# nikhilTkur/Multigrid_Nikhil_C-

Hardware: AMD Instinct MI355X
Metric: fine_grid_stencil_updates_per_sec (higher is better)
Workload: dtype f64

## Files before the change

### multigrid_nikhil_c-_amd/csrc/mgx.hip

```cpp

#include "../../include/mgx.h"
#include "mgx_bottom.hpp"
#include "mgx_kernels.hpp"
#include "mgx_launch.hpp"
#include "mgx_var.hpp"
#include "mgx_galerkin.hpp"
#include "mgx_opdep.hpp"
#include "mgx_cheby.hpp"
#include "mgx_line.hpp"
#include "mgx_small.hpp"
#include "mgx_krylov.hpp"
#include "mgx_dist_plan.hpp"

#include <chrono>
#include <unistd.h>
#include <cmath>
#include <cstdio>
#include <cstdlib>
#include <cstring>
#include <string>
#include <vector>

namespace {

using namespace mgx;

thread_local std::string g_create_error;

void log_runtime_libs(const char* where)
{
    if (env_int("MGX_LOG_RUNTIME_LIBS", 0) == 0) return;
    char buf[8192];
    if (mgx_runtime_libs(buf, sizeof buf) >= 0)
        std::fprintf(stderr, "[mgx] runtime libraries mapped at %s (pid %d):\n%s", where, (int)getpid(), buf);
}

struct Level {
    int L = 0, N = 0, rows = 0;
    long pitch = 0;
    size_t bytes = 0;
    bool f64 = true;
    void *u = nullptr, *b = nullptr, *tmp = nullptr, *r = nullptr;
    void* A[9] = {};
    void* J[9] = {};
    void* wt[8] = {nullptr, nullptr, nullptr, nullptr, nullptr, nullptr, nullptr, nullptr};
    bool nine = false;
    bool stencil_set = false;
    void* cheb = nullptr;
    double lambda_g = 0.0;
    void *line_m[2] = {nullptr, nullptr}, *line_g[2] = {nullptr, nullptr}, *line_hf = nullptr, *line_hb = nullptr;
    int line_R = 0;
    size_t esize() const { return f64 ? 8 : 4; }
};

struct EventPair { hipEvent_t a, b; int cls; long long launches; long long sweeps; hipEvent_t a_use; };

}

struct mgx_solver {
    mgx_config cfg{};
    hipStream_t stream = nullptr;
    std::vector<Level> lv;
    Level fine64;
    bool mixed = false;
    bool work_f64 = true;
    BottomDST bottom;
    double* partial = nullptr;
    long partial_cap = 0;
    double* sum_dev = nullptr;
    double* sum_host = nullptr;
    std::string err;
    int rows_per_chunk = 0;
    FuseCfg fuse{10, 0, 256, 10, 10, 1024, 10, 10};
    std::vector<EventPair> ev_used, ev_free;
    double prof_ms[MGX_PROF_COUNT] = {0};
    long long prof_launches[MGX_PROF_COUNT] = {0};
    long long prof_sweeps[MGX_PROF_COUNT] = {0};
    int last_smooth_launches = 0;
    int fold = 1;
    int use_zero_in = 1;
    int norm_blocks_ready = 0;
    double fine_updates = 0.0;
    struct CycleGraph {
        std::vector<void*> before, after;
        hipGraphExec_t exec = nullptr;
        double fine_updates = 0.0;
    };
    std::vector<CycleGraph> graphs;
    int use_graph = 1;
    bool prof_mute = false;
    bool prof_chain = false;
    hipEvent_t chain_ev = nullptr;
    int mixed_fuse = 1;
    double *var_M = nullptr, *var_inv = nullptr, *var_pm = nullptr, *var_pi = nullptr;
    bool var = false;
    bool galerkin = false;
    bool gal_built = false;
    int cycle = MGX_CYCLE_V;
    int small_visit = 1;
    int small_max_n = kSmallMaxN;
    int line_dirs = 0;
    int* line_flag = nullptr;
    int transfer = MGX_TRANSFER_BILINEAR;
    struct KrylovWs {
        void *x = nullptr, *b = nullptr;
        void *p[2] = {nullptr, nullptr}, *q = nullptr;
        void *Z[kGcrMaxRestart] = {}, *Q[kGcrMaxRestart] = {};
        double* part = nullptr;
        long part_cap = 0;
        double *sc = nullptr, *sc_host = nullptr;
        int vecs(mgx_solver* s, std::initializer_list<void**> vs, size_t bytes);
        int shared(mgx_solver* s, size_t bytes, int blocks);
        void free();
    } kry;
    struct mgx_dist* dist = nullptr;

    int fail(int code, const std::string& m) { err = m; return code; }
};

namespace {

#define HIPCHK(h, expr)                                                                  \
    do {                                                                                 \
        hipError_t e__ = (expr);                                                         \
        if (e__ != hipSuccess)                                                           \
            return (h)->fail(MGX_ERR_HIP, std::string(#expr) + ": " + hipGetErrorString(e__)); \
    } while (0)

struct Prof {
    mgx_solver* s; int idx = -1;
    Prof(mgx_solver* s_, int cls, long long launches) : s(s_)
    {
        static const bool mute_all = env_int("MGX_PROF_MUTE", 0) != 0;
        if (!s->cfg.profile || s->prof_mute || mute_all) return;
        EventPair p;
        if (!s->ev_free.empty()) { p = s->ev_free.back(); s->ev_free.pop_back(); }
        else {
            static const unsigned flags = env_int("MGX_PROF_EVENT_FLAGS", 1) ? hipEventDisableSystemFence : hipEventDefault;
            if (hipEventCreateWithFlags(&p.a, flags) != hipSuccess || hipEventCreateWithFlags(&p.b, flags) != hipSuccess) return;
        }
        p.cls = cls; p.launches = launches; p.sweeps = 0;
        p.a_use = p.a;
        if (s->prof_chain && s->chain_ev) p.a_use = s->chain_ev;
        else (void)hipEventRecord(p.a, s->stream);
        s->ev_used.push_back(p);
        idx = (int)s->ev_used.size() - 1;
    }
    void set(long long launches, long long sweeps)
    {
        if (idx >= 0) { s->ev_used[idx].launches = launches; s->ev_used[idx].sweeps = sweeps; }
    }
    ~Prof()
    {
        if (idx < 0) return;
        (void)hipEventRecord(s->ev_used[idx].b, s->stream);
        if (s->prof_chain) s->chain_ev = s->ev_used[idx].b;
    }
};

int prof_collect(mgx_solver* s)
{
    if (s->ev_used.empty()) return MGX_OK;
    HIPCHK(s, hipStreamSynchronize(s->stream));
    for (auto& p : s->ev_used) {
// ... 300 lines not shown
    s->gal_built = true;
    s->transfer = transfer;
    drop_graphs(s);
    return MGX_OK;
}

void galerkin_invalidate(mgx_solver* s)
{
    for (int lv = s->cfg.coarsest_level; lv < s->cfg.finest_level; ++lv) s->lv[lv].stencil_set = false;
    s->lv[s->cfg.finest_level].stencil_set = true;
    s->gal_built = false;
    drop_graphs(s);
}

int var_ready(mgx_solver* s, int lo, int hi)
{
    if (!s->var) return MGX_OK;
    if (s->galerkin && !s->gal_built)
        return s->fail(MGX_ERR_STATE, s->lv[s->cfg.finest_level].stencil_set ? "Galerkin hierarchy not built (mgx_build_galerkin)"
                                                                             : "finest operator not set (mgx_set_stencil / mgx_set_coefficient)");
    for (int l = lo; l <= hi; ++l)
        if (!s->lv[l].stencil_set)
            return s->fail(MGX_ERR_STATE, "operator of level " + std::to_string(l) + " not set (mgx_set_stencil / mgx_set_coefficient)");
    return MGX_OK;
}

template <typename T>
void smooth_var_t(mgx_solver* s, Level& l, int mu)
{
    const T om = (T)s->cfg.omega;
    const T rc = (T)(1.0 - (double)om);
    const Launch g = make_launch(l.N, VecOf<T>::W, l.N - 1, 1);
    const VarLevel<T> v = var_level<T>(l);
    for (int i = 0; i < mu; ++i) {
        with_point_count(v.nine, [&](auto nq) {
            hipLaunchKernelGGL((k_jacobi_var<T, decltype(nq)::value>), dim3(g.blocks), dim3(kBlock), 0, s->stream, (const T*)l.u, (const T*)l.b,
                               (T*)l.tmp, v.dinv, v.r, v.N, v.pitch, 1, v.N, g.strips, rc, om, v.rows);
        });
        std::swap(l.u, l.tmp);
    }
    s->last_smooth_launches = mu;
}

template <typename T>
void smooth_cheby_t(mgx_solver* s, Level& l, int mu)
{
    const T om = (T)s->cfg.omega;
    const T rc = (T)(1.0 - (double)om);
    const std::vector<ChebyStep> st = cheby_scalars(s->cfg.omega, l.lambda_g, mu);
    const VarLevel<T> cl = var_level<T>(l);
    for (int i = 0; i < mu; ++i) {
        launch_cheby<T>(cl, (const T*)l.u, (const T*)l.b, (T*)l.tmp, (T*)l.cheb, i == 0, rc, om, (T)st[i].a, (T)st[i].c, s->stream);
        std::swap(l.u, l.tmp);
    }
    s->last_smooth_launches = mu;
}

template <typename T>
void smooth_line_t(mgx_solver* s, Level& l, int mu)
{
    const LineLevel<T> ll = line_level<T>(l);
    int launches = 0;
    for (int i = 0; i < mu; ++i) launches += launch_line_sweep<T>(ll, (T*)l.u, (const T*)l.b, s->line_dirs, s->stream);
    s->last_smooth_launches = launches;
}

void smooth_var(mgx_solver* s, Level& l, int mu)
{
    if (s->line_dirs) { if (l.f64) smooth_line_t<double>(s, l, mu); else smooth_line_t<float>(s, l, mu); }
    else if (s->cfg.smoother == MGX_SMOOTHER_CHEBYSHEV) { if (l.f64) smooth_cheby_t<double>(s, l, mu); else smooth_cheby_t<float>(s, l, mu); }
    else if (l.f64) smooth_var_t<double>(s, l, mu);
    else smooth_var_t<float>(s, l, mu);
}

template <typename T, int MODE>
void residual_var_t(mgx_solver* s, const Level& l, const void* u, const void* b, void* out)
{
    const Launch g = make_launch(l.N, VecOf<T>::W, l.N - 1, 1);
    const VarLevel<T> v = var_level<T>(l);
    with_point_count(v.nine, [&](auto nq) {
        hipLaunchKernelGGL((k_residual_var<T, decltype(nq)::value, MODE>), dim3(g.blocks), dim3(kBlock), 0, s->stream, (const T*)u, (const T*)b,
                           (T*)out, s->partial, v.a, v.N, v.pitch, 1, v.N, g.strips, v.rows);
    });
    if (MODE == 1) hipLaunchKernelGGL(k_reduce_partials, dim3(1), dim3(kReduceThreads), 0, s->stream, s->partial, g.blocks, s->sum_dev);
}

template <int MODE>
void residual_level(mgx_solver* s, const Level& l, const void* u, const void* b, void* out)
{
    with_float_type(l.f64, [&](auto tag) {
        using T = decltype(tag);
        if (s->var) residual_var_t<T, MODE>(s, l, u, b, out);
        else launch_residual<T, MODE>((const T*)u, (const T*)b, out, MODE ? 0 : l.pitch, MODE ? s->partial : nullptr, MODE ? s->sum_dev : nullptr,
                                      1.0, l.N, l.pitch, 1, l.N, s->rows_per_chunk, s->stream, MODE ? s->partial_cap : -1, l.rows);
    });
}

template <typename T, int SM, int AR>
int fold_block(const FuseCfg& fc, const BlockReq& q, T* u, const T* b, T* tmp, long pitch, double omega, const mgx_slab* c,
               const T* coarse_e, T* coarse_b, T* coarse_zero, int crow_lo, int crow_hi, int restrict_mode, double* partial,
               hipStream_t st, int* flips)
{
    std::vector<Pass> plan;
    if (!fold_plan(fc, q, &plan)) return -1;
    const int N = q.N, row0 = q.row0;
    const JacobiCoef<T> jc = jacobi_coef<T>(omega);
    FoldArgs fa;
    fa.restrict_mode = restrict_mode;
    fa.partial = partial;
    fa.win.row_first = std::max(row0, 0);
    fa.win.row_last = std::min(row0 + q.rows - 1, N);
    fa.win.crow_first = 0; fa.win.crow_last = -1; fa.win.emit_lo = 0; fa.win.emit_hi = 0;
    if (c) {
        fa.cpitch = level_pitch(c->level, c->dtype);
        fa.win.crow_first = std::max(c->row0, 0);
        fa.win.crow_last = std::min(c->row0 + c->rows - 1, N / 2);
        fa.win.emit_lo = std::max(c->row0 + crow_lo, 1);
        fa.win.emit_hi = std::min(c->row0 + crow_hi, N / 2);
        const long cback = (long)c->row0 * fa.cpitch;
        if (coarse_e) fa.coarse_e = coarse_e - cback;
        if (coarse_b) fa.coarse_b = coarse_b - cback;
        if (coarse_zero) fa.coarse_zero = coarse_zero - cback;
    }
    const long back = (long)row0 * pitch;
    T* src = u; T* dst = tmp;
    int blocks = 0;
    for (const Pass& p : plan) {
        if (p.hi > p.lo) {
            const int lo = p.lo - row0, hi = p.hi - row0;
            fa.row_lo = p.lo; fa.row_hi = p.hi;
            fa.zero_in = p.zero_in ? 1 : 0;
            int rc = 0;
            if (p.kind == PASS_JACOBI)
                rc = launch_jacobi<T>(src, b, dst, N, pitch, lo, hi, omega, p.R, st, q.rows, AR) ? -1 : 0;
            else if (p.kind == PASS_RBGS)
                launch_rbgs<T>(src, b, dst, N, pitch, lo, hi, row0 & 1, -row0, N - row0, p.R, st);
            else if (p.kind == PASS_FUSED)
                rc = launch_fused<T, SM, AR>(p.K, src, b, dst, N, pitch, lo, hi, jc.c0, jc.c1, -row0, N - row0, row0 & 1, p.R, st,
                                             q.rows, fa.zero_in) ? 0 : -1;
            else if (p.kind == PASS_FOLDED)
                rc = with_stages(p.pre, p.post, [&](auto s) {
                    using S = decltype(s);
                    if constexpr (S::PRE || S::POST)
                        return launch_cycle<T, S::PRE, S::POST, SM, AR>(p.K, src - back, b - back, dst - back, fa, N, pitch, jc.c0, jc.c1, p.R, st);
                    else
                        return -1;
                });
            else
                rc = launch_tile_pass<T, SM, AR>(src - back, b - back, dst - back, fa, N, pitch, jc.c0, jc.c1, p.K, p.R, p.pre, p.post, st);
            if (rc < 0) return -1;
            if (p.post == 2) blocks = rc;
        }
        std::swap(src, dst);
    }
    *flips = (int)plan.size();
    return blocks;
}

bool fold_eligible(const mgx_solver* s, const Level& l, int mu, bool pre = false, int post = 1, bool zero_in = false)
{
    if (!s->fold || mu < 1 || mu > 64) return false;
    if (s->var || (post == 1 && s->cfg.restrict_mode >= MGX_RESTRICT_INJECT)) return false;
    const int per = (s->cfg.smoother == MGX_SMOOTHER_RBGS) ? 2 : 1;
    if (!tile_level(s, l) && (l.N < s->fuse.min_n || s->fuse.kmax < per)) return false;
    std::vector<Pass> plan;
    return fold_plan(s->fuse, level_req(s, l, mu, pre, post, zero_in, 0), &plan);
}

bool zero_in_ok(const mgx_solver* s, int level)
{
    if (!s->use_zero_in || level <= s->cfg.coarsest_level) return false;
    return fold_eligible(s, s->lv[level], s->cfg.mu1, false, 1, true);
}

bool smooth_folded(mgx_solver* s, int level, int mu, bool pre, int post, bool zero_in = false, bool coarse_zero_in = false)
{
    Level& l = s->lv[level];
    if (!fold_eligible(s, l, mu, pre, post)) return false;
    const bool fine = (level == s->cfg.finest_level);
    const bool rbgs = (s->cfg.smoother == MGX_SMOOTHER_RBGS);
    if (!l.f64 && !rbgs && mu == 10 && l.N > s->fuse.tile_max_n && post == 2 && pre &&
        cycle_k_supported(mu, false, false, 0, pre, s->fuse.arith) && !cycle_k_supported(mu, false, false, post, pre, s->fuse.arith))
        post = 0;
    {
        Prof p(s, fine ? MGX_PROF_SMOOTH_FINE : MGX_PROF_COARSE, mu);
        const Level& c = s->lv[level - 1];
        const int dt = l.f64 ? MGX_DTYPE_F64 : MGX_DTYPE_F32;
        const mgx_slab cs{level - 1, dt, c.rows, 0, s->cfg.arith};
        void* czero = (post == 1 && coarse_zero_in) ? nullptr : c.u;
        const BlockReq q = level_req(s, l, mu, pre, post, zero_in, env_int("MGX_ROWS", 0));
        int launches = 0;
        const int nb = with_kernel_set(l.f64, s->cfg.smoother, s->fuse.arith, [&](auto k) {
            using K = decltype(k);
            using T = typename K::T;
            return fold_block<T, K::SM, K::AR>(s->fuse, q, (T*)l.u, (const T*)l.b, (T*)l.tmp, l.pitch, s->cfg.omega, &cs,
                                               pre ? (const T*)c.u : nullptr, post == 1 ? (T*)c.b : nullptr, (T*)czero, 1, c.N,
                                               s->cfg.restrict_mode, s->partial, s->stream, &launches);
        });
        if (nb < 0) return false;
        if (launches & 1) std::swap(l.u, l.tmp);
        p.set(launches, mu);
        if (post == 2) s->norm_blocks_ready = nb;
    }
    if (fine) s->fine_updates += (double)mu * (double)(l.N - 1) * (double)(l.N - 1);
    return true;
}

void smooth_t(mgx_solver* s, Level& l, int mu)
{
    int launches = 0;
    with_kernel_set(l.f64, s->cfg.smoother, s->fuse.arith, [&](auto k) {
        using K = decltype(k);
        using T = typename K::T;
        (void)fold_block<T, K::SM, K::AR>(s->fuse, level_req(s, l, mu, false, 0, false, s->rows_per_chunk), (T*)l.u, (const T*)l.b,
                                          (T*)l.tmp, l.pitch, s->cfg.omega, nullptr, nullptr, nullptr, nullptr, 0, 0, 0, nullptr,
                                          s->stream, &launches);
    });
    s->last_smooth_launches = launches;
    if (launches & 1) std::swap(l.u, l.tmp);
}

void smooth(mgx_solver* s, int level, int mu)
{
    if (mu <= 0) return;
    Level& l = s->lv[level];
    const bool fine = (level == s->cfg.finest_level);
    Prof p(s, fine ? MGX_PROF_SMOOTH_FINE : MGX_PROF_COARSE, mu);
    if (s->var) smooth_var(s, l, mu);
    else smooth_t(s, l, mu);
    p.set(s->last_smooth_launches, mu);
    if (fine) s->fine_updates += (double)(s->line_dirs == 3 ? 2 * mu : mu) * (double)(l.N - 1) * (double)(l.N - 1);
}

void restrict_level(mgx_solver* s, int level, bool fused, bool zero_guess)
{
    Level& f = s->lv[level];
    Level& c = s->lv[level - 1];
    const bool fine = (level == s->cfg.finest_level);
    Prof p(s, fine ? MGX_PROF_RESTRICT_FINE : MGX_PROF_COARSE, 1);
    const int rpc = s->rows_per_chunk;
    const int mode = s->cfg.restrict_mode;
    with_float_type(f.f64, [&](auto tag) {
        using T = decltype(tag);
        T* cz = zero_guess ? (T*)c.u : nullptr;
        if (opdep(s)) {
            const Launch g = make_launch(c.N, VecOf<T>::W, c.N - 1, 1);
            const T rscale = (mode == MGX_RESTRICT_FW16) ? (T)0.25 : (T)1;
            const dim3 grd(g.blocks), blk(kBlock);
            if (!fused) hipLaunchKernelGGL((k_restrict_opdep<T, 0>), grd, blk, 0, s->stream, (const T*)f.u, (const T*)f.b, op9_of<T>(f), wt8_of<T>(c),
                                           (T*)c.b, cz, c.N, f.pitch, c.pitch, g.strips, rscale);
            else with_point_count(f.nine, [&](auto nq) {
                hipLaunchKernelGGL((k_restrict_opdep<T, decltype(nq)::value == 9 ? 2 : 1>), grd, blk, 0, s->stream, (const T*)f.u, (const T*)f.b,
                                   op9_of<T>(f), wt8_of<T>(c), (T*)c.b, cz, c.N, f.pitch, c.pitch, g.strips, rscale);
            });
            return;
        }
        const bool grid_residual = fused && (s->var || mode >= MGX_RESTRICT_INJECT);
        if (grid_residual) residual_level<0>(s, f, f.u, f.b, f.r);
        const T* src = (const T*)(grid_residual ? f.r : f.b);
        if (mode >= MGX_RESTRICT_INJECT) {
            const double w = (mode == MGX_RESTRICT_INJECT4) ? 4.0 : 1.0;
            const dim3 blk(256), grd((c.N + 255) / 256, c.N - 1);
            hipLaunchKernelGGL((k_restrict_inject<T>), grd, blk, 0, s->stream, src, (T*)c.b, cz, c.N, f.pitch, c.pitch, (T)w);
        } else {
            launch_restrict<T>((const T*)f.u, src, (T*)c.b, cz, f.N, f.pitch, c.pitch, 1, c.N, 0, mode, fused && !grid_residual, rpc, s->stream);
        }
    });
}

void prolong_level(mgx_solver* s, int level, bool add)
{
    Level& f = s->lv[level];
    Level& c = s->lv[level - 1];
    const bool fine = (level == s->cfg.finest_level);
    Prof p(s, fine ? MGX_PROF_PROLONG_FINE : MGX_PROF_COARSE, 1);
    with_float_type(f.f64, [&](auto tag) {
        using T = decltype(tag);
        if (!opdep(s)) {
            launch_prolong<T>((T*)f.u, (const T*)c.u, f.N, f.pitch, c.pitch, 1, f.N, 0, add, s->rows_per_chunk, s->stream);
            return;
        }
        const Launch g = make_launch(c.N, VecOf<T>::W, c.N, 1);
        if (add) hipLaunchKernelGGL((k_prolong_opdep<T, true>), dim3(g.blocks), dim3(kBlock), 0, s->stream, (T*)f.u, (const T*)c.u, wt8_of<T>(c),
                                    c.N, f.pitch, c.pitch, g.strips);
        else hipLaunchKernelGGL((k_prolong_opdep<T, false>), dim3(g.blocks), dim3(kBlock), 0, s->stream, (T*)f.u, (const T*)c.u, wt8_of<T>(c),
                                c.N, f.pitch, c.pitch, g.strips);
    });
}

void bottom_solve(mgx_solver* s)
{
    Level& l = s->lv[s->cfg.coarsest_level];
    Prof p(s, (l.L == s->cfg.finest_level) ? MGX_PROF_SMOOTH_FINE : MGX_PROF_COARSE, 4);
    const int n = l.N - 1;
    with_float_type(l.f64, [&](auto tag) {
        using T = decltype(tag);
        if (s->var)
            hipLaunchKernelGGL((k_var_dense_solve<T>), dim3((n * n + 63) / 64), dim3(64), 0, s->stream, s->var_inv, (const T*)l.b, (T*)l.u, n, l.pitch);
        else s->bottom.solve<T>((const T*)l.b, (T*)l.u, l.pitch, s->stream);
    });
}

int zero_u(mgx_solver* s, int level)
{
    Level& l = s->lv[level];
    HIPCHK(s, hipMemsetAsync(l.u, 0, l.bytes, s->stream));
    return MGX_OK;
}

bool descend(mgx_solver* s, int level, bool zero_in_here)
{
    const bool zin_next = zero_in_ok(s, level - 1);
    if (!smooth_folded(s, level, s->cfg.mu1, false, 1, zero_in_here, zin_next)) {
        if (zero_in_here) (void)zero_u(s, level);
        smooth(s, level, s->cfg.mu1);
        restrict_level(s, level, true, !zin_next);
    }
    return zin_next;
}

void ascend(mgx_solver* s, int level, int post)
{
    if (!smooth_folded(s, level, s->cfg.mu2, true, post)) {
        prolong_level(s, level, true);
        smooth(s, level, s->cfg.mu2);
    }
}

void vcycle(mgx_solver* s, int level, bool zero_in_here = false, int post_top = 0, int kind = -1);

bool small_level(const mgx_solver* s, int level)
{
    if (!s->small_visit || s->cycle == MGX_CYCLE_V || !s->galerkin || !s->gal_built) return false;
    if (s->cfg.smoother != MGX_SMOOTHER_JACOBI) return false;
    if (level <= s->cfg.coarsest_level || level > s->cfg.finest_level) return false;
    const Level& l = s->lv[level];
    return l.nine && l.N <= s->small_max_n;
}

void small_visit(mgx_solver* s, int level, bool ascend, bool descend)
{
    Level& f = s->lv[level];
    Level& c = s->lv[level - 1];
    Prof p(s, MGX_PROF_COARSE, 1);
    with_float_type(f.f64, [&](auto tag) {
        using T = decltype(tag);
        SmallVisit<T> a;
        a.u = (T*)f.u; a.b = (const T*)f.b;
        a.a = op9_of<T>(f); a.r = jac9_of<T>(f); a.dinv = (const T*)f.J[0];
        a.cu = (T*)c.u; a.cb = (T*)c.b;
        a.w = wt8_of<T>(c);
        a.N = f.N; a.pitch = f.pitch; a.cpitch = c.pitch;
        a.ascend = ascend; a.descend = descend; a.mu1 = s->cfg.mu1; a.mu2 = s->cfg.mu2;
        a.opdep = opdep(s);
        a.omega = (T)s->cfg.omega;
        a.rc = (T)(1.0 - (double)a.omega);
        const bool fw16 = s->cfg.restrict_mode == MGX_RESTRICT_FW16;
        a.rscale = fw16 ? (T)0.25 : (T)1;
        a.wgt = fw16 ? (T)0.0625 : (T)0.25;
        launch_small_visit<T>(a, s->stream);
    });
    p.set(1, (ascend ? s->cfg.mu2 : 0) + (descend ? s->cfg.mu1 : 0));
}

void coarse_visits(mgx_solver* s, int level, bool zero_in_here, int kind)
{
    const bool twice = kind != MGX_CYCLE_V && level > s->cfg.coarsest_level;
    const int second = kind == MGX_CYCLE_F ? MGX_CYCLE_V : kind;
    if (twice && small_level(s, level)) {
        small_visit(s, level, false, true);
        coarse_visits(s, level - 1, false, kind);
        small_visit(s, level, true, true);
        coarse_visits(s, level - 1, false, second);
        small_visit(s, level, true, false);
        return;
    }
    vcycle(s, level, zero_in_here, 0, kind);
    if (twice) vcycle(s, level, false, 0, second);
}

void vcycle(mgx_solver* s, int level, bool zero_in_here, int post_top, int kind)
{
    if (kind < 0) kind = s->cycle;
    if (level == s->cfg.coarsest_level) {
        if (s->cfg.bottom == MGX_BOTTOM_EXACT) {
            bottom_solve(s);
        } else {
            smooth(s, level, s->cfg.mu1);
            smooth(s, level, s->cfg.mu2);
        }
        return;
    }
    if (small_level(s, level)) {
        small_visit(s, level, false, true);
        coarse_visits(s, level - 1, false, kind);
        small_visit(s, level, true, false);
        return;
    }
    const bool zin_next = descend(s, level, zero_in_here);
    coarse_visits(s, level - 1, zin_next, kind);
    ascend(s, level, post_top);
}

int fmg(mgx_solver* s)
{
    const int lo = s->cfg.coarsest_level, hi = s->cfg.finest_level;
    for (int l = hi; l > lo; --l) restrict_level(s, l, false, false);
    if (s->cfg.bottom == MGX_BOTTOM_EXACT) {
        bottom_solve(s);
    } else {
        int rc = zero_u(s, lo);
        if (rc) return rc;
        for (int i = 0; i <= s->cfg.mu0; ++i) vcycle(s, lo);
    }
    for (int l = lo + 1; l <= hi; ++l) {
        prolong_level(s, l, false);
        for (int i = 0; i <= s->cfg.mu0; ++i) vcycle(s, l);
    }
    return MGX_OK;
}

int enqueue_norm(mgx_solver* s, const Level& l, const void* u, const void* b, int cls)
{
    if (s->norm_blocks_ready > 0 && u == s->lv[s->cfg.finest_level].u && !s->mixed) {
        Prof p(s, cls, 1);
        hipLaunchKernelGGL(k_reduce_partials, dim3(1), dim3(kReduceThreads), 0, s->stream, s->partial, s->norm_blocks_ready,
                           s->sum_dev);
    } else {
        Prof p(s, cls, 2);
        residual_level<1>(s, l, u, b, nullptr);
    }
    s->norm_blocks_ready = 0;
    HIPCHK(s, hipMemcpyAsync(s->sum_host, s->sum_dev, sizeof(double), hipMemcpyDeviceToHost, s->stream));
    return MGX_OK;
}

int residual_norm_grid(mgx_solver* s, const Level& l, const void* u, const void* b, double* out, int cls)
{
    int rc = enqueue_norm(s, l, u, b, cls);
    if (rc) return rc;
    HIPCHK(s, hipStreamSynchronize(s->stream));
    *out = std::sqrt(*s->sum_host);
    return MGX_OK;
}

constexpr size_t kMaxGraphs = 8;

std::vector<void*> buffer_state(const mgx_solver* s)
{
    std::vector<void*> v;
    for (int l = s->cfg.coarsest_level; l <= s->cfg.finest_level; ++l) { v.push_back(s->lv[l].u); v.push_back(s->lv[l].tmp); }
    return v;
}

void set_buffer_state(mgx_solver* s, const std::vector<void*>& v)
{
    size_t i = 0;
    for (int l = s->cfg.coarsest_level; l <= s->cfg.finest_level; ++l) { s->lv[l].u = v[i++]; s->lv[l].tmp = v[i++]; }
}

template <typename Body>
hipGraphExec_t cached_graph(mgx_solver* s, unsigned tag, Body&& enqueue)
{
    std::vector<void*> key = buffer_state(s);
    key.push_back(reinterpret_cast<void*>((uintptr_t)tag));
    for (auto& c : s->graphs)
        if (c.before == key) {
            set_buffer_state(s, c.after);
            s->fine_updates += c.fine_updates;
            return c.exec;
        }
    if (s->graphs.size() >= kMaxGraphs) return nullptr;
    const double fu0 = s->fine_updates;
    hipGraph_t graph = nullptr;
    hipGraphExec_t exec = nullptr;
    hipError_t e = hipStreamBeginCapture(s->stream, hipStreamCaptureModeThreadLocal);
    if (e == hipSuccess) {
        s->prof_mute = true;
        const int rc = enqueue();
        s->prof_mute = false;
        e = hipStreamEndCapture(s->stream, &graph);
        if (e == hipSuccess && rc != MGX_OK) e = hipErrorUnknown;
        if (e == hipSuccess) e = hipGraphInstantiate(&exec, graph, nullptr, nullptr, 0);
        if (graph) (void)hipGraphDestroy(graph);
    }
    if (e != hipSuccess) {
        (void)hipGetLastError();
        set_buffer_state(s, key);
        s->fine_updates = fu0;
        s->use_graph = 0;
        return nullptr;
    }
    s->graphs.push_back({key, buffer_state(s), exec, s->fine_updates - fu0});
    return exec;
}

int coarse_part_graph(mgx_solver* s, int level, bool zero_in_here)
{
    auto body = [&] { coarse_visits(s, level, zero_in_here, s->cycle); return MGX_OK; };
    const hipGraphExec_t exec = cached_graph(s, 4u | (zero_in_here ? 8u : 0u), body);
    if (!exec) return body();
    Prof p(s, MGX_PROF_COARSE, 1);
    HIPCHK(s, hipGraphLaunch(exec, s->stream));
    return MGX_OK;
}

int zero_start_u(mgx_solver* s, bool* implicit)
{
    const int L = s->cfg.finest_level;
    const bool one_level = L == s->cfg.coarsest_level;
    *implicit = zero_in_ok(s, L);
    if (*implicit) return MGX_OK;
    if (one_level && !s->mixed) return MGX_OK;
    return zero_u(s, L);
}

int enqueue_cycle(mgx_solver* s, bool want_norm, bool zero_start, bool split)
{
    struct Chain {
        mgx_solver* s;
        Chain(mgx_solver* s_, bool on) : s(s_) { s->prof_chain = on && env_int("MGX_PROF_CHAIN", 1) != 0; s->chain_ev = nullptr; }
        ~Chain() { s->prof_chain = false; s->chain_ev = nullptr; }
    } chain(s, split);
    const int L = s->cfg.finest_level;
    const int post = want_norm ? 2 : 0;
    s->norm_blocks_ready = 0;
    bool zin = false;
    if (zero_start)
        if (int rc = zero_start_u(s, &zin)) return rc;
    if (split) {
        const bool zin_next = descend(s, L, zin);
        if (int rc = coarse_part_graph(s, L - 1, zin_next)) return rc;
        ascend(s, L, post);
    } else {
        vcycle(s, L, zin, post);
    }
    return want_norm ? enqueue_norm(s, s->lv[L], s->lv[L].u, s->lv[L].b, MGX_PROF_NORM_FINE) : MGX_OK;
}

int cycle_body(mgx_solver* s, bool want_norm, bool zero_start, double* r)
{
    const bool split = s->cfg.profile == 2 && s->use_graph && !s->mixed && s->cfg.finest_level > s->cfg.coarsest_level;
    const bool whole = s->use_graph && !s->cfg.profile && !s->mixed;
    auto body = [&] { return enqueue_cycle(s, want_norm, zero_start, split); };
    const hipGraphExec_t exec = whole ? cached_graph(s, (want_norm ? 1u : 0u) | (zero_start ? 2u : 0u), body) : nullptr;
    if (exec) {
        s->norm_blocks_ready = 0;
        HIPCHK(s, hipGraphLaunch(exec, s->stream));
    } else if (int rc = body()) {
        return rc;
    }
    if (!want_norm) return MGX_OK;
    HIPCHK(s, hipStreamSynchronize(s->stream));
    *r = std::sqrt(*s->sum_host);
    return MGX_OK;
}

void finish_solve(mgx_stats* stats, double* history, int history_cap, const std::vector<double>& hist, int cycles, bool converged,
                  std::chrono::steady_clock::time_point t0, double fine_updates)
{
    if (stats) {
        stats->cycles = cycles;
        stats->initial_residual = hist.front();
        stats->final_residual = hist.back();
        stats->converged = converged ? 1 : 0;
        stats->seconds = std::chrono::duration<double>(std::chrono::steady_clock::now() - t0).count();
        stats->fine_updates = fine_updates;
        stats->history_len = (int)hist.size();
    }
    if (history)
        for (int i = 0; i < (int)hist.size() && i < history_cap; ++i) history[i] = hist[i];
}

double pow2_floor(double x)
{
    int e;
    (void)std::frexp(x, &e);
    return std::ldexp(1.0, e - 1);
}

Level* pick(mgx_solver* s, int level, int which, void** grid)
{
    Level* l = &s->lv[level];
    if (s->mixed && level == s->cfg.finest_level) l = &s->fine64;
    switch (which) {
        case MGX_VEC_U: *grid = l->u; break;
        case MGX_VEC_B: *grid = l->b; break;
        case MGX_VEC_R: *grid = l->r; break;
        default: *grid = nullptr;
    }
    return l;
}

template <typename T>
void fold_ring(std::vector<T>& b, const T* ring, size_t n)
{
    const size_t N = n + 1;
    const T* top = ring;
    const T* bot = ring + (N + 1);
    const T* lef = ring + 2 * (N + 1);
    const T* rig = lef + (N - 1);
    for (size_t j = 0; j < n; ++j) {
        b[j] += top[j + 1];
        b[(n - 1) * n + j] += bot[j + 1];
    }
    for (size_t i = 0; i < n; ++i) {
        b[i * n] += lef[i];
        b[i * n + (n - 1)] += rig[i];
    }
}

template <typename Enqueue>
int time_on_stream(mgx_solver* s, double* ms, Enqueue enqueue)
{
    hipEvent_t a = nullptr, b = nullptr;
    auto timed = [&]() -> int {
        HIPCHK(s, hipEventCreate(&a));
        HIPCHK(s, hipEventCreate(&b));
        HIPCHK(s, hipEventRecord(a, s->stream));
        enqueue();
        HIPCHK(s, hipEventRecord(b, s->stream));
        HIPCHK(s, hipEventSynchronize(b));
        HIPCHK(s, hipGetLastError());
        float f = 0.f;
        HIPCHK(s, hipEventElapsedTime(&f, a, b));
        *ms = f;
        return MGX_OK;
    };
    const int rc = timed();
    if (a) (void)hipEventDestroy(a);
    if (b) (void)hipEventDestroy(b);
    return rc;
}

}

#include "mgx_dist.hpp"

#define NO_DIST(s)                                                                        \
    if ((s)->dist) return (s)->fail(MGX_ERR_STATE, "not available on a multi-GPU handle (see mgx.h, Multi-GPU)");
// ... 33 lines not shown
        case MGX_ERR_INVALID: return "invalid argument";
        case MGX_ERR_NO_DEVICE: return "no usable HIP device";
        case MGX_ERR_HIP: return "HIP runtime error";
        case MGX_ERR_ALLOC: return "device allocation failed";
        case MGX_ERR_STATE: return "invalid state";
        default: return "unknown status";
    }
}

const char* mgx_last_error(mgx_handle h) { return h ? h->err.c_str() : g_create_error.c_str(); }

int mgx_level_n(int level) { return (level >= 1 && level < 31) ? (1 << level) - 1 : -1; }

long mgx_level_pitch(int level, int dtype)
{
    if (level < 1 || level > 20 || (dtype != MGX_DTYPE_F32 && dtype != MGX_DTYPE_F64)) return -1;
    return level_pitch(level, dtype);
}

int mgx_create(const mgx_config* cfg, mgx_handle* out)
{
    if (!cfg || !out) { g_create_error = "null argument"; return MGX_ERR_INVALID; }
    *out = nullptr;
    if (cfg->coarsest_level < 2 || cfg->finest_level < cfg->coarsest_level || cfg->finest_level > 15 ||
        cfg->mu0 < 0 || cfg->mu1 < 0 || cfg->mu2 < 0 || !(cfg->omega > 0.0 && cfg->omega < 2.0) ||
        cfg->smoother < 0 || cfg->smoother > MGX_SMOOTHER_LINE_ALT || cfg->smoother == 3 || cfg->dtype < 0 || cfg->dtype > 2 ||
        cfg->schedule < 0 || cfg->schedule > 1 || cfg->restrict_mode < 0 || cfg->restrict_mode > MGX_RESTRICT_INJECT4 ||
        cfg->bottom < 0 || cfg->bottom > 1 || cfg->arith < 0 || cfg->arith > 1 || (cfg->op != MGX_OPERATOR_POISSON && cfg->op != MGX_OPERATOR_STENCIL5 && cfg->op != MGX_OPERATOR_GALERKIN)) {
        g_create_error = "invalid configuration";
        return MGX_ERR_INVALID;
    }
    const bool galerkin = (cfg->op == MGX_OPERATOR_GALERKIN);
    const bool var = (cfg->op == MGX_OPERATOR_STENCIL5) || galerkin;
    if (cfg->bottom == MGX_BOTTOM_EXACT && cfg->coarsest_level > (var ? 5 : 8)) {
        g_create_error = var ? "exact bottom solve of a general operator (dense inverse) supports coarsest_level <= 5"
                             : "exact bottom solve supports coarsest_level <= 8";
        return MGX_ERR_INVALID;
    }
    const bool cheby = (cfg->smoother == MGX_SMOOTHER_CHEBYSHEV);
    if (cheby && !var) {
        g_create_error = "MGX_SMOOTHER_CHEBYSHEV: op = MGX_OPERATOR_STENCIL5 or MGX_OPERATOR_GALERKIN only (the constant stencil has its fused and folded passes)";
        return MGX_ERR_INVALID;
    }
    const bool line = (cfg->smoother >= MGX_SMOOTHER_LINE_X);
    if (line && (!var || cfg->dtype == MGX_DTYPE_MIXED || cfg->arith != MGX_ARITH_SEPARATE || cfg->n_gpus > 1)) {
        g_create_error = "MGX_SMOOTHER_LINE_X / LINE_Y / LINE_ALT: op = MGX_OPERATOR_STENCIL5 or MGX_OPERATOR_GALERKIN, dtype F64 or F32, arith SEPARATE, one GPU";
        return MGX_ERR_INVALID;
    }
    if (var && (cfg->dtype == MGX_DTYPE_MIXED || cfg->smoother == MGX_SMOOTHER_RBGS || cfg->arith != MGX_ARITH_SEPARATE || cfg->n_gpus > 1)) {
        g_create_error = cheby ? "MGX_SMOOTHER_CHEBYSHEV: dtype F64 or F32, arith SEPARATE, one GPU"
                       : galerkin ? "MGX_OPERATOR_GALERKIN: dtype F64 or F32, Jacobi or Chebyshev, arith SEPARATE, one GPU"
                                  : "MGX_OPERATOR_STENCIL5: dtype F64 or F32, Jacobi (MF:75-96) or Chebyshev, arith SEPARATE, one GPU";
        return MGX_ERR_INVALID;
    }
    if (galerkin && cfg->restrict_mode >= MGX_RESTRICT_INJECT) {
        g_create_error = "MGX_OPERATOR_GALERKIN: restrict_mode CONSISTENT or FW16 (R A P needs R = c P^T; injection has no variational meaning)";
        return MGX_ERR_INVALID;
    }
    if (cfg->restrict_mode >= MGX_RESTRICT_INJECT && (cfg->n_gpus > 1 || cfg->dtype == MGX_DTYPE_MIXED)) {
        g_create_error = "injection restriction (MF:122-130): single-GPU handles of dtype F64 or F32";
        return MGX_ERR_INVALID;
    }
    if (cfg->n_gpus > 1) return mgx_create_rank(cfg, -1, 1, nullptr, nullptr, out);
    log_runtime_libs("mgx_create");
    int ndev = 0;
    if (hipGetDeviceCount(&ndev) != hipSuccess || ndev <= 0 || cfg->device < 0 || cfg->device >= ndev) {
        g_create_error = "no usable HIP device (libmgx has no CPU fallback)";
        return MGX_ERR_NO_DEVICE;
    }
    if (hipSetDevice(cfg->device) != hipSuccess) { g_create_error = "hipSetDevice failed"; return MGX_ERR_HIP; }

    mgx_solver* s = new (std::nothrow) mgx_solver();
    if (!s) { g_create_error = "out of host memory"; return MGX_ERR_ALLOC; }
    s->cfg = *cfg;
    s->mixed = (cfg->dtype == MGX_DTYPE_MIXED);
    s->var = var;
    s->galerkin = galerkin;
    s->work_f64 = (cfg->dtype == MGX_DTYPE_F64);
    s->rows_per_chunk = env_int("MGX_ROWS", 0);
    s->fuse = fuse_cfg();
    s->fuse.arith = cfg->arith;
    s->fold = env_int("MGX_FOLD", 1);
    s->use_zero_in = env_int("MGX_ZERO_IN", 1);
    s->use_graph = env_int("MGX_GRAPH", 1);
    s->small_visit = env_int("MGX_SMALL_VISIT", 1);
    s->line_dirs = cfg->smoother == MGX_SMOOTHER_LINE_X ? 1 : cfg->smoother == MGX_SMOOTHER_LINE_Y ? 2 : cfg->smoother == MGX_SMOOTHER_LINE_ALT ? 3 : 0;
    int rc = MGX_OK;
    auto bail = [&](int code) { g_create_error = s->err; mgx_destroy(s); return code; };
    if (hipStreamCreate(&s->stream) != hipSuccess) { s->err = "hipStreamCreate failed"; return bail(MGX_ERR_HIP); }
    s->lv.resize(cfg->finest_level + 1);
    for (int l = cfg->coarsest_level; l <= cfg->finest_level; ++l)
        if ((rc = alloc_level(s, s->lv[l], l, s->work_f64)) != MGX_OK) return bail(rc);
    if (s->mixed && (rc = alloc_level(s, s->fine64, cfg->finest_level, true)) != MGX_OK) return bail(rc);
    if (var || cfg->restrict_mode >= MGX_RESTRICT_INJECT) {
        for (int l = cfg->coarsest_level + 1; l <= cfg->finest_level; ++l)
            if ((rc = ensure_r(s, s->lv[l])) != MGX_OK) return bail(rc);
    }
    if (galerkin && s->small_visit) {
        if (small_visit_prepare<double>() != hipSuccess || small_visit_prepare<float>() != hipSuccess) {
            s->err = "hipFuncSetAttribute failed for k_small_visit";
            return bail(MGX_ERR_HIP);
        }
    }
    if (var) {
        for (int l = cfg->coarsest_level; l <= cfg->finest_level; ++l) {
            s->lv[l].nine = galerkin && l < cfg->finest_level;
            if ((rc = var_alloc_level(s, s->lv[l])) != MGX_OK) return bail(rc);
            if (cheby) {
                Level& lv = s->lv[l];
                if (hipMalloc(&lv.cheb, lv.bytes) != hipSuccess) { s->err = "hipMalloc failed for the Chebyshev direction array"; return bail(MGX_ERR_ALLOC); }
                if (hipMemsetAsync(lv.cheb, 0, lv.bytes, s->stream) != hipSuccess) { s->err = "hipMemsetAsync failed"; return bail(MGX_ERR_HIP); }
            }
            if (line) {
                Level& lv = s->lv[l];
                lv.line_R = line_chunk_rows(lv.N, env_int("MGX_LINE_CHUNK", 0));
                std::vector<void**> arrays;
                for (int d = 0; d < 2; ++d)
                    if (s->line_dirs & (1 << d)) { arrays.push_back(&lv.line_m[d]); arrays.push_back(&lv.line_g[d]); }
                if ((s->line_dirs & 2) && line_chunks(lv.N, lv.line_R) > 1) { arrays.push_back(&lv.line_hf); arrays.push_back(&lv.line_hb); }
                for (void** p : arrays) {
                    if (hipMalloc(p, lv.bytes) != hipSuccess) { s->err = "hipMalloc failed for the line smoother's factor arrays"; return bail(MGX_ERR_ALLOC); }
                    if (hipMemsetAsync(*p, 0, lv.bytes, s->stream) != hipSuccess) { s->err = "hipMemsetAsync failed"; return bail(MGX_ERR_HIP); }
                }
            }
        }
        if (line && hipMalloc(&s->line_flag, sizeof(int)) != hipSuccess) { s->err = "hipMalloc failed for the line smoother's breakdown flag"; return bail(MGX_ERR_ALLOC); }
        if (cfg->bottom == MGX_BOTTOM_EXACT) {
            const size_t NN = (size_t)((1 << cfg->coarsest_level) - 1) * ((1 << cfg->coarsest_level) - 1);
            if (hipMalloc(&s->var_M, NN * NN * sizeof(double)) != hipSuccess || hipMalloc(&s->var_inv, NN * NN * sizeof(double)) != hipSuccess ||
                hipMalloc(&s->var_pm, NN * sizeof(double)) != hipSuccess || hipMalloc(&s->var_pi, NN * sizeof(double)) != hipSuccess) {
                s->err = "allocation of the coarsest operator's dense inverse failed";
                return bail(MGX_ERR_ALLOC);
            }
        }
    }
    s->mixed_fuse = env_int("MGX_MIXED_FUSE", 1);
    if (s->mixed && !s->mixed_fuse) { (void)hipFree(s->fine64.tmp); s->fine64.tmp = nullptr; }
    {
        const int N = 1 << cfg->finest_level;
        long cap = 0;
        for (int rpc : {s->rows_per_chunk, 1}) {
            cap = std::max(cap, sumsq_blocks<double>(N, N, rpc));
            cap = std::max(cap, sumsq_blocks<float>(N, N, rpc));
        }
        if (N <= s->fuse.tile_max_n) cap = std::max(cap, (long)((N + 31) / 32) * ((N + 39) / 40));
        s->partial_cap = cap + 8;
        if (hipMalloc(&s->partial, s->partial_cap * sizeof(double)) != hipSuccess ||
            hipMalloc(&s->sum_dev, sizeof(double)) != hipSuccess ||
            hipHostMalloc(&s->sum_host, sizeof(double)) != hipSuccess) {
            s->err = "allocation of reduction buffers failed";
            return bail(MGX_ERR_ALLOC);
        }
    }
    if (cfg->bottom == MGX_BOTTOM_EXACT && !var) {
        if (s->bottom.init((1 << cfg->coarsest_level) - 1) != hipSuccess) {
            s->err = "bottom solver allocation failed";
            return bail(MGX_ERR_ALLOC);
        }
    }
    if (hipStreamSynchronize(s->stream) != hipSuccess) { s->err = "device initialisation failed"; return bail(MGX_ERR_HIP); }
    *out = s;
    return MGX_OK;
}

int mgx_destroy(mgx_handle s)
{
    if (!s) return MGX_OK;
    if (s->dist) { dist_free(s->dist); s->dist = nullptr; }
    if (s->stream) (void)hipStreamSynchronize(s->stream);
    for (auto& l : s->lv) free_level(l);
    free_level(s->fine64);
    s->bottom.destroy();
    if (s->partial) (void)hipFree(s->partial);
    if (s->sum_dev) (void)hipFree(s->sum_dev);
    if (s->line_flag) (void)hipFree(s->line_flag);
    if (s->sum_host) (void)hipHostFree(s->sum_host);
    for (double* p : {s->var_M, s->var_inv, s->var_pm, s->var_pi}) if (p) (void)hipFree(p);
    s->kry.free();
    drop_graphs(s);
    for (auto& p : s->ev_used) { (void)hipEventDestroy(p.a); (void)hipEventDestroy(p.b); }
    for (auto& p : s->ev_free) { (void)hipEventDestroy(p.a); (void)hipEventDestroy(p.b); }
    if (s->stream) (void)hipStreamDestroy(s->stream);
    delete s;
    return MGX_OK;
}

int mgx_graphs_cached(mgx_handle s)
{
    if (!s) return MGX_ERR_INVALID;
    if (s->dist) {
        mgx_handle c = s->dist->slabs[0].coarse;
        return (c && c->use_graph) ? (int)c->graphs.size() : -1;
    }
    if (!s->use_graph || s->cfg.profile == 1 || s->mixed) return -1;
    return (int)s->graphs.size();
}

int mgx_synchronize(mgx_handle s)
{
    if (!s) return MGX_ERR_INVALID;
    if (s->dist) return dist_sync(s, s->dist);
    HIPCHK(s, hipStreamSynchronize(s->stream));
    return MGX_OK;
}

int mgx_set_level(mgx_handle s, int level, int which, const void* src, size_t count)
{
    if (!s || !src) return MGX_ERR_INVALID;
    if (!level_ok(s, level)) return s->fail(MGX_ERR_INVALID, "level out of range");
    if (s->dist) {
        if (level != s->cfg.finest_level || (which != MGX_VEC_U && which != MGX_VEC_B))
            return s->fail(MGX_ERR_STATE, "multi-GPU handles exchange U and B of the finest level only");
        return dist_set(s, s->dist, which, src, count);
    }
    void* grid = nullptr;
    Level* l = pick(s, level, which, &grid);
    if (which == MGX_VEC_R) {
        int rc = ensure_r(s, *l);
        if (rc) return rc;
        grid = l->r;
    }
    if (!grid) return s->fail(MGX_ERR_INVALID, "unknown vector selector");
    return copy_in(s, *l, grid, src, count);
}

int mgx_get_level(mgx_handle s, int level, int which, void* dst, size_t count)
{
    if (!s || !dst) return MGX_ERR_INVALID;
    if (!level_ok(s, level)) return s->fail(MGX_ERR_INVALID, "level out of range");
    if (s->dist) {
        if (level != s->cfg.finest_level || (which != MGX_VEC_U && which != MGX_VEC_B))
            return s->fail(MGX_ERR_STATE, "multi-GPU handles exchange U and B of the finest level only");
        return dist_get(s, s->dist, which, dst, count);
    }
    void* grid = nullptr;
    Level* l = pick(s, level, which, &grid);
    if (!grid) return s->fail(MGX_ERR_STATE, "vector not available (call mgx_residual first for MGX_VEC_R)");
    return copy_out(s, *l, grid, dst, count);
}

int mgx_set_level_device(mgx_handle s, int level, int which, const void* grid)
{
    if (!s || !grid) return MGX_ERR_INVALID;
    NO_DIST(s)
    if (!level_ok(s, level)) return s->fail(MGX_ERR_INVALID, "level out of range");
    void* dst = nullptr;
    Level* l = pick(s, level, which, &dst);
    if (which == MGX_VEC_R) {
        int rc = ensure_r(s, *l);
        if (rc) return rc;
        dst = l->r;
    }
    if (!dst) return s->fail(MGX_ERR_INVALID, "unknown vector selector");
    HIPCHK(s, hipMemcpyAsync(dst, grid, l->bytes, hipMemcpyDeviceToDevice, s->stream));
    HIPCHK(s, hipStreamSynchronize(s->stream));
    return MGX_OK;
}

int mgx_get_level_device(mgx_handle s, int level, int which, void* grid)
{
    if (!s || !grid) return MGX_ERR_INVALID;
    NO_DIST(s)
    if (!level_ok(s, level)) return s->fail(MGX_ERR_INVALID, "level out of range");
// ... 317 lines not shown
    (void)pick(s, level, MGX_VEC_B, &gb);
    return residual_norm_grid(s, *l, gu, gb, out, level == s->cfg.finest_level ? MGX_PROF_NORM_FINE : MGX_PROF_COARSE);
}

int mgx_vcycle(mgx_handle s, int level)
{
    if (s && s->dist) {
        if (level != s->cfg.finest_level) return s->fail(MGX_ERR_STATE, "multi-GPU handles: V-cycles from the finest level only");
        int rc = dist_vcycle(s, s->dist);
        return rc ? rc : dist_sync(s, s->dist);
    }
    OP_PROLOGUE(s->cfg.coarsest_level)
    vcycle(s, level);
    OP_EPILOGUE
}

int mgx_set_cycle(mgx_handle s, int cycle)
{
    if (!s) return MGX_ERR_INVALID;
    if (cycle != MGX_CYCLE_V && cycle != MGX_CYCLE_W && cycle != MGX_CYCLE_F)
        return s->fail(MGX_ERR_INVALID, "cycle must be MGX_CYCLE_V, MGX_CYCLE_W or MGX_CYCLE_F");
    if (s->dist) return s->fail(MGX_ERR_STATE, "mgx_set_cycle: multi-GPU handles run V-cycles only (the slab plan has no second coarse visit)");
    if (s->mixed) return s->fail(MGX_ERR_STATE, "mgx_set_cycle: dtype MIXED handles run V-cycles only; use a F64 or F32 handle");
    if (!s->var)
        return s->fail(MGX_ERR_STATE, "mgx_set_cycle: op = MGX_OPERATOR_POISSON handles run V-cycles only; W- and F-cycles are for "
                                      "MGX_OPERATOR_STENCIL5 and MGX_OPERATOR_GALERKIN");
    drop_graphs(s);
    s->cycle = cycle;
    return MGX_OK;
}

int mgx_get_cycle(mgx_handle s, int* cycle)
{
    if (!s) return MGX_ERR_INVALID;
    if (!cycle) return s->fail(MGX_ERR_INVALID, "null argument");
    *cycle = s->cycle;
    return MGX_OK;
}

int mgx_vcycle_zero(mgx_handle s)
{
    if (!s) return MGX_ERR_INVALID;
    NO_DIST(s)
    MIXED_GUARD(s->cfg.finest_level)
    if (int vr = var_ready(s, s->cfg.coarsest_level, s->cfg.finest_level)) return vr;
    double unused = 0.0;
    int rc = cycle_body(s, false, true, &unused);
    if (rc) return rc;
    OP_EPILOGUE
}

int mgx_fmg(mgx_handle s)
{
    if (!s) return MGX_ERR_INVALID;
    if (s->dist) {
        int rc = dist_fmg(s, s->dist);
        return rc ? rc : dist_sync(s, s->dist);
    }
    MIXED_GUARD(s->cfg.finest_level)
    if (int vr = var_ready(s, s->cfg.coarsest_level, s->cfg.finest_level)) return vr;
    int rc = fmg(s);
    if (rc) return rc;
    OP_EPILOGUE
}

int mgx_solve(mgx_handle s, double tol, int max_cycles, mgx_stats* stats, double* history, int history_cap)
{
    if (!s || max_cycles < 0 || !(tol >= 0.0)) return MGX_ERR_INVALID;
    if (s->dist) return dist_solve(s, s->dist, tol, max_cycles, stats, history, history_cap);
    if (int vr = var_ready(s, s->cfg.coarsest_level, s->cfg.finest_level)) return vr;
    const int L = s->cfg.finest_level;
    const bool do_fmg = (s->cfg.schedule == MGX_SCHEDULE_FMG);
    std::vector<double> hist;
    hist.reserve(max_cycles + 1);
    s->fine_updates = 0.0;
    HIPCHK(s, hipStreamSynchronize(s->stream));
    const auto t0 = std::chrono::steady_clock::now();
    int rc = MGX_OK;
    double r = 0.0;
    int k = 0;

    if (!s->mixed) {
        Level& l = s->lv[L];
        if ((rc = residual_norm_grid(s, l, l.u, l.b, &r, MGX_PROF_NORM_FINE))) return rc;
        hist.push_back(r);
        for (k = 0; k < max_cycles; ++k) {
            if (hist[k] <= tol * hist[0]) break;
            s->norm_blocks_ready = 0;
            if (k == 0 && do_fmg) {
                if ((rc = fmg(s))) return rc;
                if ((rc = residual_norm_grid(s, l, l.u, l.b, &r, MGX_PROF_NORM_FINE))) return rc;
            } else if ((rc = cycle_body(s, true, false, &r))) {
                return rc;
            }
            hist.push_back(r);
        }
    } else {
        Level& w = s->lv[L];
        Level& d = s->fine64;
        const double n = (double)(w.N - 1);
        const int rpc = s->rows_per_chunk;
        if ((rc = residual_norm_grid(s, d, d.u, d.b, &r, MGX_PROF_NORM_FINE))) return rc;
        hist.push_back(r);
        for (k = 0; k < max_cycles; ++k) {
            if (hist[k] <= tol * hist[0]) break;
            const Launch g = make_launch(d.N, 2, d.N - 1, rpc);
            double pending_scale = 0.0;
            if (k == 0 && do_fmg) {
                HIPCHK(s, hipMemsetAsync(d.u, 0, d.bytes, s->stream));
                double bn = 0.0;
                if ((rc = residual_norm_grid(s, d, d.u, d.b, &bn, MGX_PROF_NORM_FINE))) return rc;
                const double scale = pow2_floor(bn / n);
                hipLaunchKernelGGL(k_scale_f64_to_f32, dim3(g.blocks), dim3(kBlock), 0, s->stream, (float*)w.b,
                                   (const double*)d.b, 1.0 / scale, d.N, d.pitch, w.pitch, 1, d.N, g.R, g.strips, g.chunks);
                if ((rc = fmg(s))) return rc;
                hipLaunchKernelGGL(k_axpy_f32_to_f64, dim3(g.blocks), dim3(kBlock), 0, s->stream, (double*)d.u,
                                   (const float*)w.u, scale, d.N, d.pitch, w.pitch, 1, d.N, g.R, g.strips, g.chunks, 1);
            } else {
                const double scale = pow2_floor(hist[k > 0 ? k - 1 : 0] / n);
                if (k == 0) {
                    Prof p(s, MGX_PROF_NORM_FINE, 2);
                    launch_residual<double, 2>((const double*)d.u, (const double*)d.b, w.b, w.pitch, s->partial,
                                               s->sum_dev, 1.0 / scale, d.N, d.pitch, 1, d.N, rpc, s->stream, s->partial_cap, d.rows);
                }
                double unused = 0.0;
                if ((rc = cycle_body(s, false, true, &unused))) return rc;
                pending_scale = scale;
                if (!(s->mixed_fuse && d.tmp)) {
                    hipLaunchKernelGGL(k_axpy_f32_to_f64, dim3(g.blocks), dim3(kBlock), 0, s->stream, (double*)d.u,
                                       (const float*)w.u, scale, d.N, d.pitch, w.pitch, 1, d.N, g.R, g.strips, g.chunks, 0);
                    pending_scale = 0.0;
                }
            }
            {
                const double next_scale = pow2_floor(hist[k] / n);
                Prof p(s, MGX_PROF_NORM_FINE, 2);
                if (pending_scale != 0.0) {
                    static const int mixed_rows = env_int("MGX_MIXED_ROWS", 0);
                    Launch gr = make_launch(d.N, 2, d.N - 1, mixed_rows > 0 ? mixed_rows : rpc);
                    if (gr.blocks > s->partial_cap) {
                        const int R = (int)(((long)gr.strips * (d.N - 1) / kWavesPerBlock + s->partial_cap - 9) / (s->partial_cap - 8)) + 1;
                        gr = make_launch(d.N, 2, d.N - 1, R);
                    }
                    hipLaunchKernelGGL(k_update_residual, dim3(gr.blocks), dim3(kBlock), 0, s->stream, (const double*)d.u,
                                       (const float*)w.u, (const double*)d.b, (double*)d.tmp, (float*)w.b, pending_scale,
                                       1.0 / next_scale, s->partial, d.N, d.pitch, w.pitch, 1, d.N, gr.R, gr.strips, gr.chunks);
                    hipLaunchKernelGGL(k_reduce_partials, dim3(1), dim3(kReduceThreads), 0, s->stream, s->partial, gr.blocks, s->sum_dev);
                    std::swap(d.u, d.tmp);
                } else {
                    launch_residual<double, 2>((const double*)d.u, (const double*)d.b, w.b, w.pitch, s->partial,
                                               s->sum_dev, 1.0 / next_scale, d.N, d.pitch, 1, d.N, rpc, s->stream, s->partial_cap, d.rows);
                }
            }
            HIPCHK(s, hipMemcpyAsync(s->sum_host, s->sum_dev, sizeof(double), hipMemcpyDeviceToHost, s->stream));
            HIPCHK(s, hipStreamSynchronize(s->stream));
            hist.push_back(std::sqrt(*s->sum_host));
        }
    }
    HIPCHK(s, hipGetLastError());
    HIPCHK(s, hipStreamSynchronize(s->stream));
    finish_solve(stats, history, history_cap, hist, k, hist.back() <= tol * hist.front(), t0, s->fine_updates);
    return MGX_OK;
}

int mgx_solve_pcg(mgx_handle s, double tol, int max_iters, mgx_stats* stats, double* history, int history_cap)
{
    return krylov_solve(s, "mgx_solve_pcg", nullptr, tol, max_iters, stats, history, history_cap, [](auto t) { return PcgMethod<decltype(t)>{}; });
}

int mgx_solve_gcr(mgx_handle s, double tol, int max_iters, int restart, mgx_stats* stats, double* history, int history_cap)
{
    static_assert(kGcrMaxRestart == MGX_GCR_MAX_RESTART, "mgx_krylov.hpp and mgx.h disagree");
    const char* bad_restart = (restart < 1 || restart > MGX_GCR_MAX_RESTART) ? "1 <= restart <= MGX_GCR_MAX_RESTART required" : nullptr;
    return krylov_solve(s, "mgx_solve_gcr", bad_restart, tol, max_iters, stats, history, history_cap,
                        [restart](auto t) { return GcrMethod<decltype(t)>{restart}; });
}

int mgx_time_gcr_pass(mgx_handle s, int pass, int j, int repeats, double* ms)
{
    if (!s || !ms || repeats < 1 || pass < MGX_GCR_PASS_UPDATE || pass > MGX_GCR_PASS_DIRECTION || j < 0 || j >= MGX_GCR_MAX_RESTART ||
        (pass == MGX_GCR_PASS_DOTS && j == 0))
        return s ? s->fail(MGX_ERR_INVALID, "mgx_time_gcr_pass: pass, 0 <= j < MGX_GCR_MAX_RESTART (dots: j >= 1) and repeats >= 1 required")
                 : MGX_ERR_INVALID;
    NO_DIST(s)
    if (s->mixed) return s->fail(MGX_ERR_STATE, "mgx_time_gcr_pass: dtype MIXED is not supported");
    if (int vr = var_ready(s, s->cfg.coarsest_level, s->cfg.finest_level)) return vr;
    for (int i = 0; i <= j; ++i)
        if (!s->kry.Z[i] || !s->kry.Q[i] || !s->kry.x || !s->kry.sc)
            return s->fail(MGX_ERR_STATE, "mgx_time_gcr_pass: call mgx_solve_gcr with restart > j first (it allocates the basis)");
    return s->work_f64 ? gcr_time_pass<double>(s, pass, j, repeats, ms) : gcr_time_pass<float>(s, pass, j, repeats, ms);
}

int mgx_profile_reset(mgx_handle s)
{
    if (!s) return MGX_ERR_INVALID;
    if (s->dist) {
        int rc = dist_prof_collect(s, s->dist);
        if (rc) return rc;
        for (int i = 0; i < MGX_PROF_COUNT; ++i) { s->dist->prof_ms[i] = 0.0; s->dist->prof_launches[i] = 0; s->dist->prof_sweeps[i] = 0; }
        return MGX_OK;
    }
    int rc = prof_collect(s);
    if (rc) return rc;
    for (int i = 0; i < MGX_PROF_COUNT; ++i) { s->prof_ms[i] = 0.0; s->prof_launches[i] = 0; s->prof_sweeps[i] = 0; }
    return MGX_OK;
}

int mgx_profile_get(mgx_handle s, mgx_profile* out)
{
    if (!s || !out) return MGX_ERR_INVALID;
    if (s->dist) {
        int rc = dist_prof_collect(s, s->dist);
        if (rc) return rc;
        for (int i = 0; i < MGX_PROF_COUNT; ++i) {
            out->ms[i] = s->dist->prof_ms[i]; out->launches[i] = s->dist->prof_launches[i]; out->sweeps[i] = s->dist->prof_sweeps[i];
        }
        return MGX_OK;
    }
    int rc = prof_collect(s);
    if (rc) return rc;
    for (int i = 0; i < MGX_PROF_COUNT; ++i) {
        out->ms[i] = s->prof_ms[i];
        out->launches[i] = s->prof_launches[i];
        out->sweeps[i] = s->prof_sweeps[i];
    }
    return MGX_OK;
}

int mgx_time_smoother(mgx_handle s, int sweeps, double* ms)
{
    if (!s || !ms || sweeps < 1) return MGX_ERR_INVALID;
    NO_DIST(s)
    if (int vr = var_ready(s, s->cfg.finest_level, s->cfg.finest_level)) return vr;
    Level& l = s->lv[s->cfg.finest_level];
    return time_on_stream(s, ms, [&] {
        if (s->var) smooth_var(s, l, sweeps);
        else smooth_t(s, l, sweeps);
// ... 14 lines not shown
    if (slab_check(s)) return -1;
    const int N = 1 << s->level;
    const int rpc = env_int("MGX_ROWS", 0);
    long cap = 0;
    for (int r : {rpc, 1}) {
        cap = std::max(cap, sumsq_blocks<double>(N, s->rows, r));
        cap = std::max(cap, sumsq_blocks<float>(N, s->rows, r));
    }
    return cap + 8;
}

static BlockReq slab_req(const mgx_slab& s, int smoother, int row_lo, int row_hi, int mu, bool pre = false, int post = 0,
                         bool zero_in = false)
{
    BlockReq q{smoother, s.dtype == MGX_DTYPE_F64, 1 << s.level, s.row0, s.rows, row_lo, row_hi, mu, pre, post, zero_in};
    q.rpc = env_int("MGX_ROWS", 0);
    return q;
}

static int slab_smooth(int smoother, const mgx_slab* s, void* u, const void* b, void* tmp, int row_lo, int row_hi,
                       int mu, double omega, int shrink, int* result_in_tmp, void* stream)
{
    if (slab_check(s) || !u || !b || !tmp || mu < 0) return MGX_ERR_INVALID;
    FuseCfg fc = fuse_cfg();
    fc.arith = s->arith;
    BlockReq q = slab_req(*s, smoother, row_lo, row_hi, mu);
    q.widen = shrink != 0;
    q.strict = true;
    const long pitch = level_pitch(s->level, s->dtype);
    int flips = 0;
    const int rc = with_kernel_set(q.f64, smoother, s->arith, [&](auto k) {
        using K = decltype(k);
        using T = typename K::T;
        return fold_block<T, K::SM, K::AR>(fc, q, (T*)u, (const T*)b, (T*)tmp, pitch, omega, nullptr, nullptr, nullptr, nullptr,
                                           0, 0, 0, nullptr, (hipStream_t)stream, &flips);
    });
    if (rc < 0) return MGX_ERR_INVALID;
    if (result_in_tmp) *result_in_tmp = flips & 1;
    return hipGetLastError() == hipSuccess ? MGX_OK : MGX_ERR_HIP;
}

int mgx_slab_jacobi(const mgx_slab* s, void* u, const void* b, void* tmp, int row_lo, int row_hi, int mu,
                    double omega, int shrink, int* result_in_tmp, void* stream)
{
    return slab_smooth(MGX_SMOOTHER_JACOBI, s, u, b, tmp, row_lo, row_hi, mu, omega, shrink, result_in_tmp, stream);
}

int mgx_slab_rbgs(const mgx_slab* s, void* u, const void* b, void* tmp, int row_lo, int row_hi, int mu,
                  int shrink, int* result_in_tmp, void* stream)
{
    return slab_smooth(MGX_SMOOTHER_RBGS, s, u, b, tmp, row_lo, row_hi, mu, 1.0, shrink, result_in_tmp, stream);
}

int mgx_slab_cycle(const mgx_slab* f, void* u, const void* b, void* tmp, int row_lo, int row_hi, int mu, double omega,
                   int smoother, const mgx_slab* c, const void* coarse_e, void* coarse_b, int crow_lo, int crow_hi,
                   int restrict_mode, int zero_in, double* scratch, double* sum_dev, int* result_in_tmp, void* stream)
{
    if (zero_in && coarse_e) return MGX_ERR_INVALID;
    if (smoother != MGX_SMOOTHER_JACOBI && smoother != MGX_SMOOTHER_RBGS) return MGX_ERR_INVALID;
    if (restrict_mode != MGX_RESTRICT_CONSISTENT && restrict_mode != MGX_RESTRICT_FW16) return MGX_ERR_INVALID;
    if (coarse_b && !((std::max(row_lo + f->row0, 1)) & 1)) return MGX_ERR_INVALID;
    if (slab_check(f) || !u || !b || !tmp || mu < 1 || mu > 64 || row_hi <= row_lo) return MGX_ERR_INVALID;
    if ((coarse_e || coarse_b) && (slab_check(c) || c->level != f->level - 1 || c->dtype != f->dtype)) return MGX_ERR_INVALID;
    if (coarse_b && sum_dev) return MGX_ERR_INVALID;
    if (sum_dev && !scratch) return MGX_ERR_INVALID;
    if (coarse_b && (crow_lo < 0 || crow_hi > c->rows || crow_hi < crow_lo)) return MGX_ERR_INVALID;
    const int N = 1 << f->level;
    if (row_lo < 0 || row_hi > f->rows || row_lo + f->row0 < 1 || row_hi + f->row0 > N) return MGX_ERR_INVALID;
    FuseCfg fc = fuse_cfg();
    fc.arith = f->arith;
    const int post = coarse_b ? 1 : (sum_dev ? 2 : 0);
    BlockReq q = slab_req(*f, smoother, row_lo, row_hi, mu, coarse_e != nullptr, post, zero_in != 0);
    q.tile_points = env_int("MGX_SLAB_TILE_POINTS", 1 << 20);
    const long pitch = level_pitch(f->level, f->dtype);
    hipStream_t st = (hipStream_t)stream;
    int flips = 0;
    const int nb = with_kernel_set(q.f64, smoother, f->arith, [&](auto k) {
        using K = decltype(k);
        using T = typename K::T;
        return fold_block<T, K::SM, K::AR>(fc, q, (T*)u, (const T*)b, (T*)tmp, pitch, omega, c, (const T*)coarse_e,
                                           (T*)coarse_b, nullptr, crow_lo, crow_hi, restrict_mode, scratch, st, &flips);
    });
    if (nb < 0) return MGX_ERR_INVALID;
    if (post == 2) hipLaunchKernelGGL(k_reduce_partials, dim3(1), dim3(kReduceThreads), 0, st, scratch, nb, sum_dev);
    if (result_in_tmp) *result_in_tmp = flips & 1;
    return hipGetLastError() == hipSuccess ? MGX_OK : MGX_ERR_HIP;
}

int mgx_slab_restrict(const mgx_slab* f, const void* u, const void* b, const mgx_slab* c, void* cb, void* zero_u,
                      int crow_lo, int crow_hi, int restrict_mode, int fused, void* stream)
{
    if (slab_check(f) || slab_check(c) || !b || !cb || (fused && !u)) return MGX_ERR_INVALID;
    if (restrict_mode != MGX_RESTRICT_CONSISTENT && restrict_mode != MGX_RESTRICT_FW16) return MGX_ERR_INVALID;
    if (c->level != f->level - 1 || c->dtype != f->dtype) return MGX_ERR_INVALID;
    const int N = 1 << f->level;
    const long pitch = level_pitch(f->level, f->dtype), cpitch = level_pitch(c->level, c->dtype);
    const int off = 2 * c->row0 - f->row0;
    const int halo = fused ? 2 : 1;
    if (crow_lo < 0 || crow_hi > c->rows || crow_lo + c->row0 < 1 || crow_hi + c->row0 > N / 2) return MGX_ERR_INVALID;
    if (crow_hi > crow_lo && (2 * crow_lo + off - halo < 0 || 2 * (crow_hi - 1) + off + halo > f->rows - 1)) return MGX_ERR_INVALID;
    const int rpc = env_int("MGX_ROWS", 0);
    if (f->dtype == MGX_DTYPE_F64)
        launch_restrict<double>((const double*)u, (const double*)b, (double*)cb, (double*)zero_u, N, pitch, cpitch,
                                crow_lo, crow_hi, off, restrict_mode, fused != 0, rpc, (hipStream_t)stream);
    else
        launch_restrict<float>((const float*)u, (const float*)b, (float*)cb, (float*)zero_u, N, pitch, cpitch,
                               crow_lo, crow_hi, off, restrict_mode, fused != 0, rpc, (hipStream_t)stream);
    return hipGetLastError() == hipSuccess ? MGX_OK : MGX_ERR_HIP;
}

int mgx_slab_prolong(const mgx_slab* f, void* u, const mgx_slab* c, const void* e, int row_lo, int row_hi, int add,
                     void* stream)
{
    if (slab_check(f) || slab_check(c) || !u || !e) return MGX_ERR_INVALID;
    if (c->level != f->level - 1 || c->dtype != f->dtype) return MGX_ERR_INVALID;
    const int N = 1 << f->level;
    const long pitch = level_pitch(f->level, f->dtype), cpitch = level_pitch(c->level, c->dtype);
    const int off = 2 * c->row0 - f->row0;
    if (row_lo < 0 || row_hi > f->rows || row_lo + f->row0 < 1 || row_hi + f->row0 > N) return MGX_ERR_INVALID;
    if (row_hi > row_lo) {
        const int ylo = row_lo - off, yhi = row_hi - 1 - off;
        if (ylo < 0 || (yhi >> 1) + (yhi & 1) > c->rows - 1) return MGX_ERR_INVALID;
    }
    const int rpc = env_int("MGX_ROWS", 0);
    if (f->dtype == MGX_DTYPE_F64)
        launch_prolong<double>((double*)u, (const double*)e, N, pitch, cpitch, row_lo, row_hi, off, add != 0, rpc, (hipStream_t)stream);
    else
        launch_prolong<float>((float*)u, (const float*)e, N, pitch, cpitch, row_lo, row_hi, off, add != 0, rpc, (hipStream_t)stream);
    return hipGetLastError() == hipSuccess ? MGX_OK : MGX_ERR_HIP;
}

int mgx_slab_residual_sumsq(const mgx_slab* s, const void* u, const void* b, int row_lo, int row_hi,
                            double* scratch, double* sum_dev, void* stream)
{
    if (slab_check(s) || !u || !b || !scratch || !sum_dev) return MGX_ERR_INVALID;
    const int N = 1 << s->level;
    const long pitch = level_pitch(s->level, s->dtype);
    if (row_lo < 1 || row_hi > s->rows - 1 || row_lo + s->row0 < 1 || row_hi + s->row0 > N || row_hi <= row_lo) return MGX_ERR_INVALID;
    const int rpc = env_int("MGX_ROWS", 0);
    if (s->dtype == MGX_DTYPE_F64)
        launch_residual<double, 1>((const double*)u, (const double*)b, nullptr, 0, scratch, sum_dev, 1.0, N, pitch, row_lo, row_hi, rpc, (hipStream_t)stream, -1, s->rows);
    else
        launch_residual<float, 1>((const float*)u, (const float*)b, nullptr, 0, scratch, sum_dev, 1.0, N, pitch, row_lo, row_hi, rpc, (hipStream_t)stream, -1, s->rows);
    return hipGetLastError() == hipSuccess ? MGX_OK : MGX_ERR_HIP;
}

int mgx_create_rank(const mgx_config* cfg, int rank, int world, const void* rccl_id, const mgx_transport* transport,
                    mgx_handle* out)
{
    if (!cfg || !out) { g_create_error = "null argument"; return MGX_ERR_INVALID; }
    *out = nullptr;
    if (cfg->smoother == MGX_SMOOTHER_CHEBYSHEV) {
        g_create_error = "MGX_SMOOTHER_CHEBYSHEV: single-GPU handles of op = MGX_OPERATOR_STENCIL5 / MGX_OPERATOR_GALERKIN only";
        return MGX_ERR_INVALID;
    }
    if (cfg->smoother >= MGX_SMOOTHER_LINE_X && cfg->smoother <= MGX_SMOOTHER_LINE_ALT) {
        g_create_error = "MGX_SMOOTHER_LINE_X / LINE_Y / LINE_ALT: single-GPU handles of op = MGX_OPERATOR_STENCIL5 / MGX_OPERATOR_GALERKIN only";
        return MGX_ERR_INVALID;
    }
    if (cfg->coarsest_level < 2 || cfg->finest_level < cfg->coarsest_level || cfg->finest_level > 15 ||
        cfg->mu1 < 0 || cfg->mu2 < 0 || !(cfg->omega > 0.0 && cfg->omega < 2.0) || cfg->smoother < 0 || cfg->smoother > 1 ||
        cfg->dtype < 0 || cfg->dtype > 2 || cfg->restrict_mode < 0 || cfg->restrict_mode > 1 || cfg->bottom < 0 || cfg->bottom > 1 || cfg->arith < 0 || cfg->arith > 1 ||
        (rank >= 0 && (world < 1 || rank >= world)) || (rank < 0 && cfg->n_gpus < 2)) {
        g_create_error = "invalid configuration";
        return MGX_ERR_INVALID;
    }
    if (cfg->op != MGX_OPERATOR_POISSON) {
// ... 155 lines not shown
```

### multigrid_nikhil_c-_amd/csrc/mgx_inst.hip

```cpp
#include "mgx_launch.hpp"
#if MGX_INST_KIND == 4
#include "mgx_cheby.hpp"
#elif MGX_INST_KIND == 5
#include "mgx_small.hpp"
#elif MGX_INST_KIND == 6
#include "mgx_line.hpp"
#elif MGX_INST_KIND == 7
#include "mgx_krylov.hpp"
#endif

namespace mgx {
using T_ = MGX_INST_T;
#if MGX_INST_KIND == 1
#if MGX_INST_PP == 0
#define PP_ 1, 2
#elif MGX_INST_PP == 1
#define PP_ 1, 0
#elif MGX_INST_PP == 2
#define PP_ 0, 1
#elif MGX_INST_PP == 3
#define PP_ 0, 2
#else
#define PP_ 1, 1
#endif
template int launch_cycle<T_, PP_, MGX_INST_SM, MGX_INST_AR>(int, const T_*, const T_*, T_*, const FoldArgs&, int, long, T_, T_, int, hipStream_t);
#elif MGX_INST_KIND == 2
template bool launch_fused<T_, MGX_INST_SM, MGX_INST_AR>(int, const T_*, const T_*, T_*, int, long, int, int, T_, T_, int, int, int, int, hipStream_t, int, int);
#elif MGX_INST_KIND == 3
template int launch_tile_pass<T_, MGX_INST_SM, MGX_INST_AR>(const T_*, const T_*, T_*, const FoldArgs&, int, long, T_, T_, int, int, bool, int, hipStream_t);
#elif MGX_INST_KIND == 4
template void launch_cheby<T_>(const VarLevel<T_>&, const T_*, const T_*, T_*, T_*, bool, T_, T_, T_, T_, hipStream_t);
template void launch_lambda_max<T_>(const VarLevel<T_>&, double*, long, double*, hipStream_t);
#elif MGX_INST_KIND == 5
template hipError_t small_visit_prepare<T_>();
template void launch_small_visit<T_>(const SmallVisit<T_>&, hipStream_t);
#elif MGX_INST_KIND == 6
template void launch_line_factor<T_>(const LineLevel<T_>&, int, int*, hipStream_t);
template int launch_line_sweep<T_>(const LineLevel<T_>&, T_*, const T_*, int, hipStream_t);
#elif MGX_INST_KIND == 7
template void launch_gcr_orth<T_>(int, T_*, T_*, const T_*, const GcrBasis<T_>&, double*, double*, int, long, const Launch&, int, hipStream_t);
#else
#error "MGX_INST_KIND must be 1 .. 7"
#endif
}
```

### multigrid_nikhil_c-_amd/csrc/mgx_kernels.hpp

```cpp
#pragma once

#include <hip/hip_runtime.h>
#include "mgx_geom.hpp"
#include <stdint.h>
#include <type_traits>

namespace mgx {

template <int B, int E, typename F> __device__ __forceinline__ void static_for(F&& f)
{
    if constexpr (B < E) {
        f(std::integral_constant<int, B>{});
        static_for<B + 1, E>(f);
    }
}

constexpr int kWave = 64;
constexpr int kBlock = 256;
constexpr int kWavesPerBlock = kBlock / kWave;
constexpr int kOutLanes = kWave - 2;

template <typename T> struct VecOf;
template <> struct VecOf<double> { using type = double2; static constexpr int W = 2; };
template <> struct VecOf<float>  { using type = float4;  static constexpr int W = 4; };
// ... 552 lines not shown
    fo.lane_off = (unsigned)(col * (long)sizeof(T));
    fo.clane_off = 0;
    if (interior) {
        if (zero_in) fused_body<T, K, SM, false, true, AR>(pv, pb, po, pitch, col, N, r0, r1, true, st, c0, c1, bnd_lo, bnd_hi, rd_lo, rd_hi, row_parity, true, fo);
        else fused_body<T, K, SM, false, false, AR>(pv, pb, po, pitch, col, N, r0, r1, true, st, c0, c1, bnd_lo, bnd_hi, rd_lo, rd_hi, row_parity, false, fo);
    } else {
        fused_body<T, K, SM, true, false, AR>(pv, pb, po, pitch, col, N, r0, r1, ld, st, c0, c1, bnd_lo, bnd_hi, rd_lo, rd_hi, row_parity, zero_in != 0, fo);
    }
}

template <int K, int W> constexpr int fused_out_lanes() { return kWave - 2 * ((K + W - 1) / W); }

__device__ __forceinline__ double2 residual_vec(const double2& up, const double2& cur, const double2& dn, const double2& bb)
{
    const double l = from_left(cur.y), r = from_right(cur.x);
    double2 o;
    o.x = bb.x - (-nbr(up.x, l, cur.y, dn.x) + 4.0 * cur.x);
    o.y = bb.y - (-nbr(up.y, cur.x, r, dn.y) + 4.0 * cur.y);
    return o;
}
__device__ __forceinline__ float4 residual_vec(const float4& up, const float4& cur, const float4& dn, const float4& bb)
{
    const NbrPairs t = nbr_pairs(up, cur, dn);
    const f32x2 p0 = {cur.x, cur.y}, p1 = {cur.z, cur.w}, b0 = {bb.x, bb.y}, b1 = {bb.z, bb.w};
    const f32x2 o0 = b0 - (-t.t0 + 4.f * p0);
    const f32x2 o1 = b1 - (-t.t1 + 4.f * p1);
    return make_float4(o0.x, o0.y, o1.x, o1.y);
}

template <typename T, int MODE>
__global__ void __launch_bounds__(kBlock)
k_residual(const T* __restrict__ vin, const T* __restrict__ rhs, void* __restrict__ out, long pitch_out,
           double* __restrict__ partial, double inv_scale,
           int N, long pitch, int row_lo, int row_hi, int R, int strips, int chunks, int rows_alloc)
{
    using V = typename VecOf<T>::type;
    constexpr int W = VecOf<T>::W;
    __shared__ double wsum[kWavesPerBlock];
    const Tile t = wave_tile(strips, chunks);
    double acc = 0.0;
    if (t.active) {
        const Cols c = lane_cols<W>(t.strip, N, pitch);
        const int r0 = row_lo + t.chunk * R;
        const int r1 = min(r0 + R, row_hi);
        const T* pv = vin + c.col;
        const T* pb = rhs + c.col;
        auto has = [&](int y) { return c.ld && y >= 0 && y < rows_alloc; };
        V up = vload<V>(pv + (long)(r0 - 1) * pitch, has(r0 - 1));
        V cur = vload<V>(pv + (long)r0 * pitch, has(r0));
        for (int r = r0; r < r1; ++r) {
            const V dn = vload<V>(pv + (long)(r + 1) * pitch, has(r + 1));
            const V bb = vload<V>(pb + (long)r * pitch, has(r));
            V o = residual_vec(up, cur, dn, bb);
            mask_cols(o, c.col, N);
            if (MODE == 0) {
                vstore<V>(reinterpret_cast<T*>(out) + c.col + (long)r * pitch, o, c.st);
            } else {
                if (c.st) {
                    if constexpr (W == 2) acc += (double)o.x * (double)o.x + (double)o.y * (double)o.y;
                    else acc += ((double)o.x * (double)o.x + (double)o.y * (double)o.y) +
                                ((double)o.z * (double)o.z + (double)o.w * (double)o.w);
                }
                if constexpr (MODE == 2 && W == 2) {
                    float2 f = make_float2((float)(o.x * inv_scale), (float)(o.y * inv_scale));
                    if (c.st) *reinterpret_cast<float2*>(reinterpret_cast<float*>(out) + c.col + (long)r * pitch_out) = f;
                }
            }
            up = cur; cur = dn;
        }
    }
    if (MODE != 0) {
        for (int off = 32; off > 0; off >>= 1) acc += __shfl_down(acc, off, kWave);
        if ((threadIdx.x & 63) == 0) wsum[threadIdx.x >> 6] = acc;
        __syncthreads();
        if (threadIdx.x == 0) {
            double s = 0.0;
            for (int w = 0; w < kWavesPerBlock; ++w) s += wsum[w];
            partial[blockIdx.x] = s;
        }
    }
}

constexpr int kReduceThreads = 1024;
static __global__ void __launch_bounds__(kReduceThreads) k_reduce_partials(const double* __restrict__ partial, int n, double* __restrict__ out)
{
    __shared__ double wsum[kReduceThreads / kWave];
    double a0 = 0.0, a1 = 0.0, a2 = 0.0, a3 = 0.0;
    int i = threadIdx.x;
    for (; i + 3 * kReduceThreads < n; i += 4 * kReduceThreads) {
        a0 += partial[i];
        a1 += partial[i + kReduceThreads];
        a2 += partial[i + 2 * kReduceThreads];
        a3 += partial[i + 3 * kReduceThreads];
    }
    for (; i < n; i += kReduceThreads) a0 += partial[i];
    double acc = (a0 + a1) + (a2 + a3);
    for (int off = 32; off > 0; off >>= 1) acc += __shfl_down(acc, off, kWave);
    if ((threadIdx.x & 63) == 0) wsum[threadIdx.x >> 6] = acc;
    __syncthreads();
    if (threadIdx.x == 0) {
        double s = 0.0;
        for (int w = 0; w < kReduceThreads / kWave; ++w) s += wsum[w];
        out[0] = s;
    }
}

struct ReduceSum { __device__ __forceinline__ double operator()(double a, double b) const { return a + b; } };
struct ReduceMax { __device__ __forceinline__ double operator()(double a, double b) const { return b > a ? b : a; } };
template <int NW, typename OP>
__device__ __forceinline__ void block_reduce(double acc, double* wsum, double* __restrict__ out, OP op)
{
    for (int off = 32; off > 0; off >>= 1) acc = op(acc, __shfl_down(acc, off, kWave));
    if ((threadIdx.x & 63) == 0) wsum[threadIdx.x >> 6] = acc;
    __syncthreads();
    if (threadIdx.x == 0) {
        double s = 0.0;
        for (int w = 0; w < NW; ++w) s = op(s, wsum[w]);
        *out = s;
    }
}

template <typename T> struct Trip { T l, c, r; };

template <typename T> __device__ __forceinline__ T restrict_fw_value(const Trip<T>& top, const Trip<T>& mid, const Trip<T>& bot, T wgt)
{
    T corners = top.l + top.r; corners = corners + bot.l; corners = corners + bot.r;
    T edges = mid.l + mid.r; edges = edges + top.c; edges = edges + bot.c;
    return wgt * ((corners + (T)2 * edges) + (T)4 * mid.c);
}
template <typename T> __device__ __forceinline__ T prolong_edge_value(T a, T b) { return (T)0.5 * (a + b); }
template <typename T> __device__ __forceinline__ T prolong_centre_value(T nw, T sw, T ne, T se) { return (T)0.25 * (((nw + sw) + ne) + se); }

template <typename T, bool FUSED>
__global__ void __launch_bounds__(kBlock)
k_restrict(const T* __restrict__ vin, const T* __restrict__ rhs, T* __restrict__ coarse, T* __restrict__ coarse_zero,
           int N, long pitch, long cpitch, int crow_lo, int crow_hi, int fine_row_off,
           int R, int strips, int chunks, T wgt)
{
    using V = typename VecOf<T>::type;
    constexpr int W = VecOf<T>::W;
    constexpr int CW = W / 2;
    const Tile t = wave_tile(strips, chunks);
    if (!t.active) return;
    const Cols c = lane_cols<W>(t.strip, N, pitch);
    const int I0 = crow_lo + t.chunk * R;
    const int I1 = min(I0 + R, crow_hi);
    const T* pv = vin + c.col;
    const T* pb = rhs + c.col;
    const long ccol = c.col / 2;
    const int NC = N / 2;

    auto row_plain = [&](int y) -> V { V o = vload<V>(pb + (long)y * pitch, c.ld); mask_cols(o, c.col, N); return o; };

    V up, cur, dn;
    int yf = 2 * I0 + fine_row_off - 1;
    if (FUSED) {
        up = vload<V>(pv + (long)(yf - 1) * pitch, c.ld);
        cur = vload<V>(pv + (long)yf * pitch, c.ld);
    }
    auto next_field = [&](int y) -> V {
        if (FUSED) {
            dn = vload<V>(pv + (long)(y + 1) * pitch, c.ld);
            const V bb = vload<V>(pb + (long)y * pitch, c.ld);
            V o = residual_vec(up, cur, dn, bb);
            mask_cols(o, c.col, N);
            up = cur; cur = dn;
            return o;
        } else {
            return row_plain(y);
        }
    };
    auto trips = [&](const V& f, Trip<T>* tr) {
        const T l = from_left(last(f));
        if constexpr (W == 2) { tr[0] = {l, f.x, f.y}; }
        else { tr[0] = {l, f.x, f.y}; tr[1] = {f.y, f.z, f.w}; }
    };

    Trip<T> top[CW], mid[CW], bot[CW];
    { const V f = next_field(yf); trips(f, top); }
    for (int I = I0; I < I1; ++I) {
        const int y = 2 * I + fine_row_off;
        { const V f = next_field(y); trips(f, mid); }
        { const V f = next_field(y + 1); trips(f, bot); }
        T o[CW];
#pragma unroll
        for (int k = 0; k < CW; ++k) {
// ... 103 lines not shown
        const unsigned srow_a = (unsigned)(Ia - fo.crb) * fo.cpitch_bytes, srow_b = (unsigned)(Ib - fo.crb) * fo.cpitch_bytes;
#pragma unroll
        for (int k = 0; k <= CW; ++k) pe.a[k] = bload1_s((T*)nullptr, fo.ce, fo.clane_off + (unsigned)(k * sizeof(T)), srow_a);
#pragma unroll
        for (int k = 0; k <= CW; ++k) pe.b[k] = bload1_s((T*)nullptr, fo.ce, fo.clane_off + (unsigned)(k * sizeof(T)), srow_b);
    } else {
        const bool cl = cld && y > 0 && y < N && I >= win.crow_first && I + (y & 1) <= win.crow_last;
        const bool cl2 = cl && (y & 1);
        const unsigned at = (unsigned)(I - fo.crb) * fo.cpitch_bytes + fo.clane_off;
#pragma unroll
        for (int k = 0; k <= CW; ++k) pe.a[k] = bload1((T*)nullptr, fo.ce, cl ? at + (unsigned)(k * sizeof(T)) : kOobOffset);
#pragma unroll
        for (int k = 0; k <= CW; ++k) pe.b[k] = bload1((T*)nullptr, fo.ce, cl2 ? at + fo.cpitch_bytes + (unsigned)(k * sizeof(T)) : kOobOffset);
    }
}

template <typename T, bool EDGE>
__device__ __forceinline__ void
coarse_row(T (&e)[VecOf<T>::W / 2 + 1], int I, bool cld, const CycleWin& win, const FastOut& fo)
{
    constexpr int CW = VecOf<T>::W / 2;
    if constexpr (!EDGE) {
        const int Ic = min(max(I, win.crow_first), win.crow_last);
        const unsigned srow = (unsigned)(Ic - fo.crb) * fo.cpitch_bytes;
#pragma unroll
        for (int k = 0; k <= CW; ++k) e[k] = bload1_s((T*)nullptr, fo.ce, fo.clane_off + (unsigned)(k * sizeof(T)), srow);
    } else {
        const bool ok = cld && I >= win.crow_first && I <= win.crow_last;
        const unsigned at = (unsigned)(I - fo.crb) * fo.cpitch_bytes + fo.clane_off;
#pragma unroll
        for (int k = 0; k <= CW; ++k) e[k] = bload1((T*)nullptr, fo.ce, ok ? at + (unsigned)(k * sizeof(T)) : kOobOffset);
    }
}

template <typename T, bool EDGE, bool ZIN = false>
__device__ __forceinline__ void
cycle_loads(typename VecOf<T>::type& in, typename VecOf<T>::type& bn, int y,
            const T* __restrict__ pv, const T* __restrict__ pb, long pitch, int N, int y_end, bool ld, bool zero_in,
            const CycleWin& win, const FastOut& fo)
{
    using V = typename VecOf<T>::type;
    if constexpr (!EDGE) {
        const int yi = min(y, win.row_last), yb = max(min(y - 1, win.row_last), win.row_first);
        if constexpr (ZIN) in = vzero((V*)nullptr);
        else in = bload_s((V*)nullptr, fo.in, fo.lane_off, (unsigned)(yi - fo.rb) * fo.pitch_bytes);
        bn = bload_s((V*)nullptr, fo.rhs, fo.lane_off, (unsigned)(yb - fo.rb) * fo.pitch_bytes);
    } else {
        const bool in_ok = !zero_in && y >= win.row_first && y <= win.row_last && y < y_end;
        const bool b_ok = (y - 1) > 0 && (y - 1) < N && (y - 1) >= win.row_first && (y - 1) <= win.row_last && y <= y_end;
        in = bload((V*)nullptr, fo.in, (ld && in_ok) ? (unsigned)(y - fo.rb) * fo.pitch_bytes + fo.lane_off : kOobOffset);
        bn = bload((V*)nullptr, fo.rhs, (ld && b_ok) ? (unsigned)(y - 1 - fo.rb) * fo.pitch_bytes + fo.lane_off : kOobOffset);
    }
}

constexpr int kBRing = 12;
template <typename T, int K, int POST, int SM> constexpr bool cycle_b_in_lds() { return (sizeof(T) == 8 && K >= 8) || (sizeof(T) == 4 && K >= 10); }
static_assert(kBRing % 2 == 0, "the deep bodies' step parity needs an even trip");
template <typename T, int K, int POST, int SM> constexpr int cycle_par() { return cycle_b_in_lds<T, K, POST, SM>() ? ((1 + K + (POST ? 1 : 0)) & 1) : -1; }
template <typename T, int K, int POST, int SM> __device__ __forceinline__ int cycle_y0(int r0)
{
    constexpr int PAR = cycle_par<T, K, POST, SM>();
    const int y0 = r0 - K - (POST ? 1 : 0);
    return PAR < 0 ? y0 : y0 - ((y0 - PAR) & 1);
}
#ifndef MGX_SKEW
#define MGX_SKEW 0
#endif
#ifndef MGX_RING_AHEAD
#define MGX_RING_AHEAD 1
#endif
#ifndef MGX_PRIO_ALT
#define MGX_PRIO_ALT 0
#endif
template <typename T, int K, int PRE, int POST, int SM, int AR> constexpr int cycle_skew()
{
    if (sizeof(T) == 8 && K == 10 && PRE == 1 && POST == 0 && SM == 0 && AR == 0) return 0;
    if (sizeof(T) == 4 && K == 10 && PRE == 0 && POST == 1 && SM == 0) return 0;
    return (MGX_SKEW != 0 && cycle_b_in_lds<T, K, POST, SM>()) ? K / 2 : 0;
}
constexpr int kRawLds = 6;
#ifndef MGX_RAWQ
#define MGX_RAWQ 1
#endif
template <typename T, int K, int PRE, int POST, int SM, int AR> constexpr bool cycle_rawq();
template <typename T> struct LdsVec;
template <> struct LdsVec<double> { typedef double v __attribute__((ext_vector_type(2))); };
template <> struct LdsVec<float> { typedef float v __attribute__((ext_vector_type(4))); };
template <typename T> using lds_vec_ptr = __attribute__((address_space(3))) typename LdsVec<T>::v*;
__device__ __forceinline__ void ring_put(lds_vec_ptr<double> r, int slot, const double2& v)
{
    LdsVec<double>::v t = {v.x, v.y};
    r[slot * kWave] = t;
}
__device__ __forceinline__ double2 ring_get(lds_vec_ptr<double> r, int slot)
{
    const LdsVec<double>::v t = r[slot * kWave];
    return make_double2(t.x, t.y);
}
__device__ __forceinline__ void ring_put(lds_vec_ptr<float> r, int slot, const float4& v)
{
    LdsVec<float>::v t = {v.x, v.y, v.z, v.w};
    r[slot * kWave] = t;
}
__device__ __forceinline__ float4 ring_get(lds_vec_ptr<float> r, int slot)
{
    const LdsVec<float>::v t = r[slot * kWave];
    return make_float4(t.x, t.y, t.z, t.w);
}
constexpr int ring_slot(int m) { return ((m % kBRing) + kBRing) % kBRing; }
template <typename T, int K, int PRE, int POST, int SM, int AR> constexpr bool cycle_rawq()
{
    if (MGX_RAWQ == 0) return false;
    if (PRE != 0 || sizeof(T) != 8) return false;
    if (POST == 2 && AR == 0 && K == 10) return false;
    return cycle_b_in_lds<T, K, POST, SM>() && SM == 0 && POST != 0 && K > kRawLds && cycle_skew<T, K, PRE, POST, SM, AR>() == 0;
}
#ifndef MGX_PFD_DEEP
#define MGX_PFD_DEEP 0
#endif
template <bool BL, int POST, bool EDGE = false> constexpr int cycle_pfd()
{
    if (BL && !EDGE && MGX_PFD_DEEP > 0) return MGX_PFD_DEEP;
    return (BL && (POST == 1 || EDGE)) ? 2 : kPrefetch;
}
constexpr int kPrefetchMax = MGX_PFD_DEEP > kPrefetch ? MGX_PFD_DEEP : kPrefetch;
template <typename T, bool BL, bool EDGE, int POST> constexpr int cycle_cpfd() { return (BL && !(EDGE && POST == 0)) ? cycle_pfd<BL, POST, EDGE>() : 1; }

template <typename T, int K, int PRE, int POST, int SM, bool EDGE, int RP, bool BL, bool ZIN, int AR, int YP>
__device__ __forceinline__ void
cycle_step(typename VecOf<T>::type (&lev)[K + 1][3], typename VecOf<T>::type (&bw)[BL ? 1 : K + 1], lds_vec_ptr<T> ring,
           lds_vec_ptr<T> ring2, typename VecOf<T>::type (&rawq)[cycle_rawq<T, K, PRE, POST, SM, AR>() ? kBRing : 1],
           typename VecOf<T>::type (&nin)[kPfStages], typename VecOf<T>::type (&nbn)[kPfStages], PreFetch<T, VecOf<T>::W / 2>& pe,
           CycleState<T, VecOf<T>::W / 2>& cs, int y,
           const T* __restrict__ pv, const T* __restrict__ pb, T* __restrict__ po,
           const T* __restrict__ coarse_e, T* __restrict__ coarse_b, T* __restrict__ coarse_zero, T wgt,
           long pitch, long col, long ccol, int N, const CycleArgs& ca, bool ld, bool cld, bool st, T c0, T c1,
           const FastOut& fo)
{
    using V = typename VecOf<T>::type;
    constexpr int W = VecOf<T>::W;
    constexpr int CW = W / 2;
    constexpr int P = RP % 3;
    constexpr int S_OLD = (P + 1) % 3, S_MID = (P + 2) % 3, S_NEW = P;
    constexpr int bnd_lo = 0;
    const int bnd_hi = N;
    const int r0 = ca.r0, r1 = ca.r1;

    if constexpr (EDGE) __builtin_amdgcn_sched_barrier(0);
    V in = nin[0];
    const V bn = nbn[0];
#pragma unroll
    for (int q = 0; q + 1 < kPfStages; ++q) { nin[q] = nin[q + 1]; nbn[q] = nbn[q + 1]; }
    cycle_loads<T, EDGE, ZIN>(nin[kPfStages - 1], nbn[kPfStages - 1], y + cycle_pfd<BL, POST, EDGE>(), pv, pb, pitch, N, ca.y_end, ld, ca.zero_in, ca.win, fo);
    const ColMask cm = col_mask(col, N);
    if (PRE) {
        T o[W];
        bool row_zero = false;
        if constexpr (YP < 0) {
            T a[CW + 1], b2[CW + 1];
#pragma unroll
            for (int k = 0; k <= CW; ++k) { a[k] = pe.a[k]; b2[k] = pe.b[k]; }
            coarse_loads<T, EDGE>(pe, y + cycle_cpfd<T, BL, EDGE, POST>(), coarse_e, ca.cpitch, ccol, N, cld, ca.win, fo);
            const bool even = (y & 1) == 0;
#pragma unroll
            for (int k = 0; k < CW; ++k) {
                const T ab = a[k] + b2[k];
                const T ev1 = (T)0.5 * (a[k] + a[k + 1]);
                const T od0 = (T)0.5 * ab;
                const T od1 = (T)0.25 * ((ab + a[k + 1]) + b2[k + 1]);
                o[2 * k] = even ? a[k] : od0;
                o[2 * k + 1] = even ? ev1 : od1;
            }
        } else {
            constexpr int CPFD = cycle_cpfd<T, BL, EDGE, POST>();
            T b2[CW + 1];
            if constexpr (YP == 1) {
#pragma unroll
                for (int k = 0; k <= CW; ++k) b2[k] = pe.b[k];
            }
            if constexpr (((YP + CPFD) & 1) == 1) coarse_row<T, EDGE>(pe.b, ((y + CPFD) >> 1) + 1, cld, ca.win, fo);
#pragma unroll
            for (int k = 0; k < CW; ++k) {
                if constexpr (YP == 0) {
                    o[2 * k] = cs.ea[k];
                    o[2 * k + 1] = (T)0.5 * (cs.ea[k] + cs.ea[k + 1]);
                } else {
                    const T ab = cs.ea[k] + b2[k];
                    o[2 * k] = (T)0.5 * ab;
                    o[2 * k + 1] = (T)0.25 * ((ab + cs.ea[k + 1]) + b2[k + 1]);
                }
            }
            if constexpr (YP == 1) {
#pragma unroll
                for (int k = 0; k <= CW; ++k) cs.ea[k] = b2[k];
            }
            if constexpr (EDGE) {
                const int I = y >> 1;
                row_zero = !(y > 0 && y < N && I >= ca.win.crow_first && I + YP <= ca.win.crow_last);
            }
        }
        V add;
        if constexpr (W == 2) add = make_double2(o[0], o[1]);
        else add = make_float4(o[0], o[1], o[2], o[3]);
        if constexpr (EDGE) mask_sel(add, cm, row_zero);
        if constexpr (W == 2) { in.x = in.x + add.x; in.y = in.y + add.y; }
        else { in.x = in.x + add.x; in.y = in.y + add.y; in.z = in.z + add.z; in.w = in.w + add.w; }
    }
    constexpr bool RAWQ = cycle_rawq<T, K, PRE, POST, SM, AR>();
    constexpr bool PREMUL = (SM == 0 && POST == 0) || RAWQ;
    V b0;
    if constexpr (PREMUL) b0 = vscale(c1, bn);
    else b0 = bn;
    if constexpr (BL) {
        asm volatile("" : "+v"(ring));
        ring_put(ring, ring_slot(RP), b0);
        if constexpr (RAWQ) {
            asm volatile("" : "+v"(ring2));
            rawq[ring_slot(RP)] = ring_get(ring2, RP % kRawLds);
            ring_put(ring2, RP % kRawLds, bn);
        }
    } else {
#pragma unroll
        for (int j = K; j > 0; --j) bw[j] = bw[j - 1];
        bw[0] = b0;
    }
    constexpr int kRingAhead = MGX_RING_AHEAD;
    constexpr int SK = cycle_skew<T, K, PRE, POST, SM, AR>();
    constexpr int SKD = SK > 0 ? 1 : 0;
    constexpr int MLAST = ((POST && !RAWQ) ? K : K - 1) + SKD;
    V rq[BL ? K + 2 : 1];
    auto bwin = [&](auto jc) -> V {
        constexpr int j = decltype(jc)::value;
        if constexpr (j == 0) return b0;
        else if constexpr (BL) return rq[j];
        else return bw[j];
    };
    V dying = lev[SK][S_NEW];
    lev[0][S_NEW] = in;
    auto level = [&](auto jc, auto bc) {
        constexpr int j = decltype(jc)::value;
        constexpr bool inB = decltype(bc)::value;
        const int row = y - j - (inB ? 1 : 0);
        const V cb = bwin(std::integral_constant<int, j - 1 + (inB ? 1 : 0)>{});
        const V& lo = (inB && j == SK + 1) ? dying : lev[j - 1][S_OLD];
        const V& mi = (inB && j == SK + 1) ? lev[j - 1][S_OLD] : lev[j - 1][S_MID];
        const V& hi = (inB && j == SK + 1) ? lev[j - 1][S_MID] : lev[j - 1][S_NEW];
        V o;
        if constexpr (PREMUL) o = jacobi_vec_pre<AR>(lo, mi, hi, cb, c0, c1);
        else o = level_op<T, SM, AR>(j, lo, mi, hi, cb, c0, c1, row + (int)(col & 1));
        if constexpr (EDGE) {
            const int rw = opaque_s(row);
            mask_sel(o, cm, !(rw > bnd_lo && rw < bnd_hi));
        }
        if constexpr (j == K) {
            const unsigned at = (unsigned)(row - fo.rb) * fo.pitch_bytes + fo.lane_off;
            bstore(o, fo.out, (st && row >= r0 && row < r1) ? at : kOobOffset);
        }
        if (j < K || POST) lev[j][S_NEW] = o;
    };
    if constexpr (SK == 0) {
        if constexpr (BL) {
            static_for<1, (kRingAhead < MLAST ? kRingAhead : MLAST) + 1>([&](auto mc) {
                constexpr int m = decltype(mc)::value;
                rq[m] = ring_get(ring, ring_slot(RP - m));
            });
        }
        static_for<1, K + 1>([&](auto jc) {
            constexpr int j = decltype(jc)::value;
            if constexpr (BL && j + kRingAhead <= MLAST) {
                rq[j + kRingAhead] = ring_get(ring, ring_slot(RP - (j + kRingAhead)));
                __builtin_amdgcn_sched_barrier(0);
            }
            level(jc, std::false_type{});
        });
    } else {
        constexpr int NB = K - SK;
        constexpr int NP = SK > NB ? SK : NB;
        rq[SK + 1] = ring_get(ring, ring_slot(RP - (SK + 1)));
        static_for<1, NP + 1>([&](auto ic) {
            constexpr int i = decltype(ic)::value;
            if constexpr (i + 1 <= SK) rq[i] = ring_get(ring, ring_slot(RP - i));
            if constexpr (i + 1 <= NB) rq[SK + i + 1] = ring_get(ring, ring_slot(RP - (SK + i + 1)));
            if constexpr (POST != 0 && i == NP) rq[K + 1] = ring_get(ring, ring_slot(RP - (K + 1)));
            __builtin_amdgcn_sched_barrier(0);
            if constexpr (i <= SK) level(std::integral_constant<int, i>{}, std::false_type{});
            if constexpr (i <= NB) level(std::integral_constant<int, SK + i>{}, std::true_type{});
        });
    }
    if (POST) {
        const int rho = y - K - 1 - SKD;
        V rawb;
        if constexpr (RAWQ) rawb = rawq[ring_slot(RP - (K - kRawLds))];
        else rawb = bwin(std::integral_constant<int, K + SKD>{});
        V res = residual_vec(lev[K][S_OLD], lev[K][S_MID], lev[K][S_NEW], rawb);
        if constexpr (EDGE) {
            const int rw = opaque_s(rho);
            mask_sel(res, cm, !(rw > bnd_lo && rw < bnd_hi));
        }
        if (POST == 2) {
            double r2;
            if constexpr (W == 2) r2 = (double)res.x * (double)res.x + (double)res.y * (double)res.y;
            else r2 = ((double)res.x * (double)res.x + (double)res.y * (double)res.y) +
                      ((double)res.z * (double)res.z + (double)res.w * (double)res.w);
            cs.acc += (st && rho >= r0 && rho < r1) ? r2 : 0.0;
        } else {
            T cl[CW], cc[CW], cr[CW];
            const T l = from_left(last(res));
            if constexpr (W == 2) { cl[0] = l; cc[0] = res.x; cr[0] = res.y; }
            else { cl[0] = l; cc[0] = res.x; cr[0] = res.y; cl[1] = res.y; cc[1] = res.z; cr[1] = res.w; }
            constexpr int RHOP = YP < 0 ? -1 : ((YP + K + 1 + SKD) & 1);
            const int I = (rho - 1) >> 1;
            if constexpr (RHOP < 0) {
                const bool odd = (rho & 1) != 0;
                const bool emit = odd && (2 * I >= r0) && (2 * I < r1) && I >= ca.win.emit_lo && I < ca.win.emit_hi;
                T o[CW];
#pragma unroll
                for (int k = 0; k < CW; ++k) {
                    T corners = cs.ct[k] + cl[k]; corners = corners + cr[k];
                    const T edges = cs.em[k] + cc[k];
                    o[k] = wgt * ((corners + (T)2 * edges) + (T)4 * cs.mc[k]);
                    if constexpr (EDGE) o[k] = (ccol + k == 0 || ccol + k >= ca.NC) ? (T)0 : o[k];
                }
                {
                    const unsigned at = (st && emit) ? ((unsigned)(I - fo.crb) * fo.cpitch_bytes + fo.clane_off) : kOobOffset;
                    if constexpr (CW == 1) { bstore8(o[0], fo.cb, at); bstore8((T)0, fo.cz, at); }
                    else { bstore8(make_float2((float)o[0], (float)o[1]), fo.cb, at); bstore8(make_float2(0.f, 0.f), fo.cz, at); }
                }
#pragma unroll
                for (int k = 0; k < CW; ++k) {
                    const T lr = cl[k] + cr[k];
                    const T em = lr + cs.tc[k];
                    cs.em[k] = odd ? cs.em[k] : em;
                    cs.mc[k] = odd ? cs.mc[k] : cc[k];
                    cs.ct[k] = odd ? lr : cs.ct[k];
                    cs.tc[k] = odd ? cc[k] : cs.tc[k];
                }
            } else if constexpr (RHOP == 1) {
                auto close_row = [&](bool emit) {
                    T o[CW];
#pragma unroll
                    for (int k = 0; k < CW; ++k) {
                        T corners = cs.ct[k] + cl[k]; corners = corners + cr[k];
                        const T edges = cs.em[k] + cc[k];
                        o[k] = wgt * ((corners + (T)2 * edges) + (T)4 * cs.mc[k]);
                        if constexpr (EDGE) o[k] = (ccol + k == 0 || ccol + k >= ca.NC) ? (T)0 : o[k];
                    }
                    const unsigned at = (st && emit) ? ((unsigned)(I - fo.crb) * fo.cpitch_bytes + fo.clane_off) : kOobOffset;
                    if constexpr (CW == 1) { bstore8(o[0], fo.cb, at); bstore8((T)0, fo.cz, at); }
                    else { bstore8(make_float2((float)o[0], (float)o[1]), fo.cb, at); bstore8(make_float2(0.f, 0.f), fo.cz, at); }
                };
                close_row((2 * I >= r0) && (2 * I < r1) && I >= ca.win.emit_lo && I < ca.win.emit_hi);
#pragma unroll
                for (int k = 0; k < CW; ++k) { cs.ct[k] = cl[k] + cr[k]; cs.tc[k] = cc[k]; }
            } else {
#pragma unroll
                for (int k = 0; k < CW; ++k) { cs.em[k] = (cl[k] + cr[k]) + cs.tc[k]; cs.mc[k] = cc[k]; }
            }
        }
    }
}

template <typename T, int K, int PRE, int POST, int SM, bool EDGE, bool ZIN, int AR>
__device__ __forceinline__ double
cycle_body(const T* __restrict__ pv, const T* __restrict__ pb, T* __restrict__ po,
           const T* __restrict__ coarse_e, T* __restrict__ coarse_b, T* __restrict__ coarse_zero, T wgt,
           long pitch, long cpitch, long col, int N, int r0, int r1, bool ld, bool st, T c0, T c1, bool zero_in,
           const CycleWin& win, lds_vec_ptr<T> ring, lds_vec_ptr<T> ring2, const FastOut& fo)
{
    constexpr bool BL = cycle_b_in_lds<T, K, POST, SM>();
    constexpr bool RAWQ = cycle_rawq<T, K, PRE, POST, SM, AR>();
    using V = typename VecOf<T>::type;
    constexpr int W = VecOf<T>::W;
    constexpr int CW = W / 2;
    constexpr int EBOT = POST == 1 ? 2 : (POST == 2 ? 1 : 0);
    const V Z = vzero((V*)nullptr);
    const long ccol = col / 2;
    const bool cld = ld && (ccol + CW < cpitch);
    V lev[K + 1][3];
    V bw[BL ? 1 : K + 1];
#pragma unroll
    for (int j = 0; j <= K; ++j) { lev[j][0] = Z; lev[j][1] = Z; lev[j][2] = Z; }
#pragma unroll
    for (int j = 0; j < (BL ? 1 : K + 1); ++j) bw[j] = Z;
    if constexpr (BL) {
#pragma unroll
        for (int q = 0; q < kBRing; ++q) ring_put(ring, q, Z);
    }
    V rawq[RAWQ ? kBRing : 1];
#pragma unroll
    for (int q = 0; q < (RAWQ ? kBRing : 1); ++q) rawq[q] = Z;
    if constexpr (RAWQ) {
#pragma unroll
        for (int q = 0; q < kRawLds; ++q) ring_put(ring2, q, Z);
    }
    CycleState<T, CW> cs;
    cs.acc = 0.0;
#pragma unroll
    for (int k = 0; k < CW; ++k) cs.ct[k] = cs.tc[k] = cs.em[k] = cs.mc[k] = (T)0;
#pragma unroll
    for (int k = 0; k <= CW; ++k) cs.ea[k] = (T)0;
    CycleArgs ca;
    ca.cpitch = cpitch; ca.NC = N / 2; ca.r0 = r0; ca.r1 = r1; ca.zero_in = zero_in; ca.win = win;
    constexpr int PAR = cycle_par<T, K, POST, SM>();
    const int y0 = cycle_y0<T, K, POST, SM>(r0);
    ca.y_end = r1 + K + EBOT + (cycle_skew<T, K, PRE, POST, SM, AR>() > 0 ? 1 : 0);
    constexpr int kRound = BL ? kBRing : trip_steps<T>();
    const int steps = (ca.y_end - y0 + kRound - 1) / kRound * kRound;
    constexpr int PFD = cycle_pfd<BL, POST, EDGE>();
    V nin[PFD][kPfStages], nbn[PFD][kPfStages];
    constexpr int CPFD = cycle_cpfd<T, BL, EDGE, POST>();
    PreFetch<T, CW> pe[CPFD];
#pragma unroll
    for (int q = 0; q < CPFD; ++q) {
#pragma unroll
        for (int k = 0; k <= CW; ++k) { pe[q].a[k] = (T)0; pe[q].b[k] = (T)0; }
    }
#pragma unroll
    for (int q = 0; q < PFD; ++q)
        cycle_loads<T, EDGE, ZIN>(nin[q][0], nbn[q][0], y0 + q, pv, pb, pitch, N, ca.y_end, ld, ca.zero_in, ca.win, fo);
    if (PRE) {
        if constexpr (PAR < 0) {
#pragma unroll
            for (int q = 0; q < CPFD; ++q) coarse_loads<T, EDGE>(pe[q], y0 + q, coarse_e, cpitch, ccol, N, cld, ca.win, fo);
        } else {
            coarse_row<T, EDGE>(cs.ea, y0 >> 1, cld, ca.win, fo);
#pragma unroll
            for (int q = 0; q < CPFD; ++q)
                if (((PAR + q) & 1) == 1) coarse_row<T, EDGE>(pe[q].b, ((y0 + q) >> 1) + 1, cld, ca.win, fo);
        }
    }
#define MGX_CSTEP(RP, Y) cycle_step<T, K, PRE, POST, SM, EDGE, RP, BL, ZIN, AR, (PAR < 0 ? -1 : ((PAR + (RP)) & 1))>(lev, bw, ring, ring2, rawq, nin[(RP) % PFD], nbn[(RP) % PFD], pe[(RP) % CPFD], cs, Y, pv, pb, po, coarse_e, coarse_b, coarse_zero, wgt, pitch, col, ccol, N, ca, ld, cld, st, c0, c1, fo)
    if constexpr (BL) {
#define MGX_CTRIP(Y) do { MGX_CSTEP(0, Y); MGX_CSTEP(1, Y + 1); MGX_CSTEP(2, Y + 2); MGX_CSTEP(3, Y + 3); MGX_CSTEP(4, Y + 4); \
                          MGX_CSTEP(5, Y + 5); MGX_CSTEP(6, Y + 6); MGX_CSTEP(7, Y + 7); MGX_CSTEP(8, Y + 8); MGX_CSTEP(9, Y + 9); \
                          MGX_CSTEP(10, Y + 10); MGX_CSTEP(11, Y + 11); } while (0)
#if MGX_PRIO_ALT
        unsigned hw_id;
        asm volatile("s_getreg_b32 %0, hwreg(HW_REG_HW_ID)" : "=s"(hw_id));
        int turn = (int)(hw_id & 1u);
        for (int y = y0; y < y0 + steps; y += kBRing) {
            if (turn & 1) __builtin_amdgcn_s_setprio(1); else __builtin_amdgcn_s_setprio(0);
            turn ^= 1;
            MGX_CTRIP(y);
        }
        __builtin_amdgcn_s_setprio(0);
#else
        for (int y = y0; y < y0 + steps; y += kBRing) MGX_CTRIP(y);
#endif
#undef MGX_CTRIP
    } else if constexpr (trip_steps<T>() == 12) {
        for (int y = y0; y < y0 + steps; y += 12) {
            MGX_CSTEP(0, y); MGX_CSTEP(1, y + 1); MGX_CSTEP(2, y + 2);
            MGX_CSTEP(3, y + 3); MGX_CSTEP(4, y + 4); MGX_CSTEP(5, y + 5);
            MGX_CSTEP(6, y + 6); MGX_CSTEP(7, y + 7); MGX_CSTEP(8, y + 8);
            MGX_CSTEP(9, y + 9); MGX_CSTEP(10, y + 10); MGX_CSTEP(11, y + 11);
        }
    } else {
        for (int y = y0; y < y0 + steps; y += 3) {
            MGX_CSTEP(0, y); MGX_CSTEP(1, y + 1); MGX_CSTEP(2, y + 2);
        }
    }
#undef MGX_CSTEP
    return cs.acc;
}

template <typename T, int K, int PRE, int POST, int SM, int AR> constexpr int cycle_waves()
{
    return cycle_b_in_lds<T, K, POST, SM>() ? 2 : 1;
}
template <typename T, int K, int PRE, int POST, int SM = 0, int AR = 0>
__global__ void __launch_bounds__(kBlock, (cycle_waves<T, K, PRE, POST, SM, AR>()))
k_jacobi_cycle(const T* __restrict__ vin, const T* __restrict__ rhs, T* __restrict__ vout,
               const T* __restrict__ coarse_e,
               T* __restrict__ coarse_b, T* __restrict__ coarse_zero, T wgt,
               double* __restrict__ partial,
               int N, long pitch, long cpitch, int row_lo, int row_hi, int R, int strips, int chunks, int Re, int chunks_e,
               int row_last0, int Rl, int RB, int n_tall, int n_short, int Rf, T c0, T c1, int zero_in, CycleWin win)
{
    constexpr int W = VecOf<T>::W;
    constexpr int XC = cycle_halo_cols<K, POST>();
    constexpr int HL = (XC + W - 1) / W;
    constexpr int OUT = kWave - 2 * HL;
    constexpr int ETOP = POST ? 1 : 0;
    constexpr int EBOT = POST == 1 ? 2 : (POST == 2 ? 1 : 0);
    __shared__ double wsum[kWavesPerBlock];
    constexpr bool BL = cycle_b_in_lds<T, K, POST, SM>();
    __shared__ typename LdsVec<T>::v bring[BL ? kWavesPerBlock * kBRing * kWave : 1];
    constexpr bool RAWQ = cycle_rawq<T, K, PRE, POST, SM, AR>();
    __shared__ typename LdsVec<T>::v braw[RAWQ ? kWavesPerBlock * kRawLds * kWave : 1];
    const CTile t = cycle_tile(strips, chunks, chunks_e, R, Re, row_lo, row_hi, row_last0, Rl, RB, n_tall, n_short, Rf);
    double acc = 0.0;
#ifdef MGX_WAVE_TRACE
    const long long trace_t0 = wall_clock64();
#endif
    if (t.active) {
        const int lane = threadIdx.x & 63;
        const int wv = __builtin_amdgcn_readfirstlane(threadIdx.x >> 6);
        lds_vec_ptr<T> ring = (lds_vec_ptr<T>)&bring[BL ? (wv * kBRing * kWave + lane) : 0];
        lds_vec_ptr<T> ring2 = (lds_vec_ptr<T>)&braw[RAWQ ? (wv * kRawLds * kWave + lane) : 0];
        const int vx0 = t.strip * OUT - HL;
        const int vx = vx0 + lane;
        const long col = (long)vx * W;
        const bool ld = (vx >= 0) && (col + W <= pitch);
        const bool st = (lane >= HL) && (lane < kWave - HL) && (vx < N / W);
        const int r0 = t.r0, r1 = t.r1;
        constexpr int kRound = BL ? kBRing : trip_steps<T>();
        const int y_first = cycle_y0<T, K, POST, SM>(r0) - 1;
        constexpr int SKD = cycle_skew<T, K, PRE, POST, SM, AR>() > 0 ? 1 : 0;
        const int y_lastp = (r0 - K - ETOP) + ((r1 + K + EBOT + SKD) - (r0 - K - ETOP) + kRound - 1) / kRound * kRound + kPrefetchMax;
        const int y0c = r0 - K - ETOP, y1c = r1 + K + EBOT - 1;
        bool interior = (vx0 >= 1) && ((long)(vx0 + kWave + 1) * W < N) &&
                        (y0c > 0) && (y1c < N) && (y0c >= win.row_first) && (y1c <= win.row_last);
        interior = interior && (y_first + 1 >= win.row_first);
        if (PRE) interior = interior && (y0c >> 1) >= win.crow_first && ((y1c + 1) >> 1) <= win.crow_last;
        interior = interior && !(PRE != 0 && zero_in);
        FastOut fo;
        fo.rb = max(y_first, win.row_first);
        fo.crb = max(y_first >> 1, win.crow_first);
        fo.pitch_bytes = (unsigned)(pitch * (long)sizeof(T));
        fo.cpitch_bytes = (unsigned)(cpitch * (long)sizeof(T));
        const unsigned f_bytes = rsrc_bytes(fo.rb, win.row_last, fo.pitch_bytes);
        const unsigned c_bytes = rsrc_bytes(fo.crb, win.crow_last, fo.cpitch_bytes);
        const long f_at = (long)fo.rb * pitch, c_at = (long)fo.crb * cpitch;
        fo.out = make_rsrc(vout + f_at, f_bytes);
        fo.in = make_rsrc(vin + f_at, f_bytes);
        fo.rhs = make_rsrc(rhs + f_at, f_bytes);
        fo.ce = make_rsrc(PRE ? coarse_e + c_at : nullptr, (PRE && coarse_e) ? c_bytes : 0u);
        fo.cb = make_rsrc((POST == 1 && coarse_b) ? coarse_b + c_at : nullptr, (POST == 1 && coarse_b) ? c_bytes : 0u);
        fo.cz = make_rsrc((POST == 1 && coarse_zero) ? coarse_zero + c_at : nullptr, (POST == 1 && coarse_zero) ? c_bytes : 0u);
        fo.lane_off = (unsigned)(col * (long)sizeof(T));
        fo.clane_off = (unsigned)((col / 2) * (long)sizeof(T));
        if (interior) {
            if (PRE == 0 && zero_in)
                acc = cycle_body<T, K, PRE, POST, SM, false, PRE == 0, AR>(vin + col, rhs + col, vout + col, coarse_e, coarse_b, coarse_zero, wgt,
                                                                      pitch, cpitch, col, N, r0, r1, true, st, c0, c1, true, win, ring, ring2, fo);
            else
                acc = cycle_body<T, K, PRE, POST, SM, false, false, AR>(vin + col, rhs + col, vout + col, coarse_e, coarse_b, coarse_zero, wgt,
                                                                    pitch, cpitch, col, N, r0, r1, true, st, c0, c1, false, win, ring, ring2, fo);
        } else {
            acc = cycle_body<T, K, PRE, POST, SM, true, false, AR>(vin + col, rhs + col, vout + col, coarse_e, coarse_b, coarse_zero, wgt,
                                                        pitch, cpitch, col, N, r0, r1, ld, st, c0, c1, zero_in != 0, win, ring, ring2, fo);
        }
    }
#ifdef MGX_WAVE_TRACE
    if ((threadIdx.x & 63) == 0) {
        const int w = blockIdx.x * kWavesPerBlock + (threadIdx.x >> 6);
        if (w < (1 << 16)) {
            unsigned hw, xcc;
            asm volatile("s_getreg_b32 %0, hwreg(HW_REG_HW_ID)" : "=s"(hw));
            asm volatile("s_getreg_b32 %0, hwreg(HW_REG_XCC_ID)" : "=s"(xcc));
            g_wave_trace[w] = WaveTrace{trace_t0, wall_clock64(), t.active ? t.strip : -1, t.r0, t.r1,
                                        (int)((hw & 0xFFF0FFFFu) | ((xcc & 0xFu) << 16))};
        }
        if (w == 0) g_wave_trace_n = gridDim.x * kWavesPerBlock;
    }
#endif
    if (POST == 2) {
        for (int off = 32; off > 0; off >>= 1) acc += __shfl_down(acc, off, kWave);
        if ((threadIdx.x & 63) == 0) wsum[threadIdx.x >> 6] = acc;
        __syncthreads();
        if (threadIdx.x == 0) {
            double sum = 0.0;
            for (int w = 0; w < kWavesPerBlock; ++w) sum += wsum[w];
            partial[blockIdx.x] = sum;
        }
    }
}

constexpr int kTileBand = 14;
constexpr int kTileSY = kWavesPerBlock * kTileBand;
constexpr int kTileSX = kWave;

template <int POST> constexpr int tile_extra() { return POST == 1 ? 2 : (POST == 2 ? 1 : 0); }

template <typename T, int SM, int PRE, int POST, int AR = 0>
__global__ void __launch_bounds__(kBlock)
k_tile_smooth(const T* __restrict__ vin, const T* __restrict__ rhs, T* __restrict__ vout,
              const T* __restrict__ coarse_e, T* __restrict__ coarse_b, T* __restrict__ coarse_zero, T wgt,
              double* __restrict__ partial, int N, long pitch, long cpitch, int levels, T c0, T c1,
              int tiles_x, int zero_in, int row_lo, int row_hi, CycleWin win)
{
    constexpr int RW = kTileBand;
    __shared__ T edge[2][kWavesPerBlock][2][kWave];
    __shared__ double wsum[kWavesPerBlock];
    const int He = levels + tile_extra<POST>();
    const int TH = kTileSY - 2 * He, TW = kTileSX - 2 * He;
    const int lane = threadIdx.x & 63;
    const int wv = __builtin_amdgcn_readfirstlane(threadIdx.x >> 6);
    const int ty = blockIdx.x / tiles_x, tx = blockIdx.x - ty * tiles_x;
    const int y0 = wv * RW;
    const int gy0 = row_lo + ty * TH - He + y0;
    const int gx = 1 + tx * TW - He + lane;
    const bool colunk = gx > 0 && gx < N;
    const int NC = N / 2;

    T u[RW], b[RW];
    unsigned rowmask = 0;
#pragma unroll
    for (int i = 0; i < RW; ++i) {
        const int gy = gy0 + i;
        const bool rowok = gy > 0 && gy < N && gy >= win.row_first && gy <= win.row_last;
        if (rowok) rowmask |= 1u << i;
        const bool unk = colunk && rowok;
        const long at = (long)gy * pitch + gx;
        u[i] = (unk && !zero_in) ? vin[at] : (T)0;
        b[i] = unk ? rhs[at] : (T)0;
    }
    if (PRE) {
        const bool codd = (gx & 1) != 0;
#pragma unroll
        for (int i = 0; i < RW; ++i) {
            const int gy = gy0 + i;
            const bool rodd = (gy & 1) != 0;
            const bool unk = colunk && ((rowmask >> i) & 1u) && (gy >> 1) >= win.crow_first && (gy >> 1) + (rodd ? 1 : 0) <= win.crow_last;
            const T* e = coarse_e + (long)(gy >> 1) * cpitch + (gx >> 1);
            const T a00 = unk ? e[0] : (T)0;
            const T a01 = (unk && codd) ? e[1] : (T)0;
            const T a10 = (unk && rodd) ? e[cpitch] : (T)0;
            const T a11 = (unk && rodd && codd) ? e[cpitch + 1] : (T)0;
            const T ev = codd ? (T)0.5 * (a00 + a01) : a00;
            const T od = codd ? (T)0.25 * (((a00 + a10) + a01) + a11) : (T)0.5 * (a00 + a10);
            const T add = rodd ? od : ev;
            u[i] = unk ? u[i] + add : u[i];
        }
    }

    int buf = 0;
    auto halo_rows = [&](const T (&a)[RW], T& up, T& dn) {
        edge[buf][wv][0][lane] = a[0];
        edge[buf][wv][1][lane] = a[RW - 1];
        __syncthreads();
        up = wv > 0 ? edge[buf][wv - 1][1][lane] : (T)0;
        dn = wv < kWavesPerBlock - 1 ? edge[buf][wv + 1][0][lane] : (T)0;
        buf ^= 1;
    };
    for (int j = 1; j <= levels; ++j) {
        T up, dn;
        halo_rows(u, up, dn);
        const bool colact = colunk && lane >= j && lane < kTileSX - j;
        const int ilo = max(j - y0, 0), ihi = min(kTileSY - j - y0, RW);
// ... 415 lines not shown
```

### multigrid_nikhil_c-_amd/csrc/mgx_launch.hpp

```cpp
#pragma once

#include "../../include/mgx.h"
#include "mgx_kernels.hpp"
#include "mgx_pass_plan.hpp"

#include <algorithm>

namespace mgx {

inline long level_pitch(int level, int dtype)
{
    const long N = 1L << level;
    const long align = (dtype == MGX_DTYPE_F64) ? 32 : 64;
    return (N + 1 + align - 1) / align * align;
}

template <typename T> struct JacobiCoef { T c0, c1; };
template <typename T>
JacobiCoef<T> jacobi_coef(double omega)
{
    const T om = (T)omega;
    return {(T)(1.0 - (double)om), (T)((double)om / 4.0)};
}

// ... 22 lines not shown
        return MGX_OK;
    }
    const Launch g = make_launch(N, VecOf<T>::W, row_hi - row_lo, rpc);
    if (arith) hipLaunchKernelGGL((k_jacobi<T, 1>), dim3(g.blocks), dim3(kBlock), 0, st, vin, b, vout, N, pitch,
                                  row_lo, row_hi, g.R, g.strips, g.chunks, c0, c1, rows_alloc);
    else hipLaunchKernelGGL((k_jacobi<T, 0>), dim3(g.blocks), dim3(kBlock), 0, st, vin, b, vout, N, pitch,
                            row_lo, row_hi, g.R, g.strips, g.chunks, c0, c1, rows_alloc);
    return MGX_OK;
}

template <typename T>
void launch_rbgs(const T* vin, const T* b, T* vout, int N, long pitch, int row_lo, int row_hi,
                 int row_parity, int bnd_lo, int bnd_hi, int rpc, hipStream_t st)
{
    if (row_hi <= row_lo) return;
    const Launch g = make_launch(N, VecOf<T>::W, row_hi - row_lo, rpc);
    hipLaunchKernelGGL((k_rbgs<T>), dim3(g.blocks), dim3(kBlock), 0, st, vin, b, vout, N, pitch,
                       row_lo, row_hi, g.R, g.strips, g.chunks, row_parity, bnd_lo, bnd_hi);
}

template <typename T, int K, int SM, int AR>
void launch_fused_k(const T* vin, const T* b, T* vout, int N, long pitch, int row_lo, int row_hi,
                    T c0, T c1, int bnd_lo, int bnd_hi, int row_parity, int R, hipStream_t st, int rows_alloc, int zero_in)
{
    constexpr int OUT = fused_out_lanes<K, VecOf<T>::W>();
    R = trip_rows(R, 2 * K, trip_steps<T>(), 1);
    Launch g = make_launch(N, VecOf<T>::W, row_hi - row_lo, R);
    g.strips = (N / VecOf<T>::W + OUT - 1) / OUT;
    const long waves = (long)g.strips * g.chunks;
    g.blocks = (int)(((waves + kWavesPerBlock - 1) / kWavesPerBlock + 7) / 8 * 8);
    hipLaunchKernelGGL((k_jacobi_fused<T, K, SM, AR>), dim3(g.blocks), dim3(kBlock), 0, st, vin, b, vout, N, pitch,
                       row_lo, row_hi, g.R, g.strips, g.chunks, c0, c1, bnd_lo, bnd_hi, row_parity, rows_alloc, zero_in);
}

template <typename T, int SM, int AR>
bool launch_fused(int K, const T* vin, const T* b, T* vout, int N, long pitch, int row_lo, int row_hi,
                  T c0, T c1, int bnd_lo, int bnd_hi, int row_parity, int R, hipStream_t st, int rows_alloc, int zero_in)
{
    switch (K) {
        case 2: launch_fused_k<T, 2, SM, AR>(vin, b, vout, N, pitch, row_lo, row_hi, c0, c1, bnd_lo, bnd_hi, row_parity, R, st, rows_alloc, zero_in); return true;
        case 4: launch_fused_k<T, 4, SM, AR>(vin, b, vout, N, pitch, row_lo, row_hi, c0, c1, bnd_lo, bnd_hi, row_parity, R, st, rows_alloc, zero_in); return true;
        case 6: launch_fused_k<T, 6, SM, AR>(vin, b, vout, N, pitch, row_lo, row_hi, c0, c1, bnd_lo, bnd_hi, row_parity, R, st, rows_alloc, zero_in); return true;
        case 8: launch_fused_k<T, 8, SM, AR>(vin, b, vout, N, pitch, row_lo, row_hi, c0, c1, bnd_lo, bnd_hi, row_parity, R, st, rows_alloc, zero_in); return true;
        case 10: launch_fused_k<T, 10, SM, AR>(vin, b, vout, N, pitch, row_lo, row_hi, c0, c1, bnd_lo, bnd_hi, row_parity, R, st, rows_alloc, zero_in); return true;
        default: break;
    }
    if constexpr (SM == 0) {
        switch (K) {
            case 3: launch_fused_k<T, 3, 0, AR>(vin, b, vout, N, pitch, row_lo, row_hi, c0, c1, bnd_lo, bnd_hi, row_parity, R, st, rows_alloc, zero_in); return true;
            case 5: launch_fused_k<T, 5, 0, AR>(vin, b, vout, N, pitch, row_lo, row_hi, c0, c1, bnd_lo, bnd_hi, row_parity, R, st, rows_alloc, zero_in); return true;
            default: break;
        }
    }
    return false;
}

struct FoldArgs {
    const void* coarse_e = nullptr;
    void* coarse_b = nullptr;
    void* coarse_zero = nullptr;
    int restrict_mode = 0;
    double* partial = nullptr;
    long cpitch = 0;
    int zero_in = 0;
    int row_lo = 0, row_hi = 0;
    CycleWin win{0, 0, 0, 0, 0, 0};
};

inline GeomKnobs geom_knobs()
{
    GeomKnobs k;
    k.edge_short = env_int("MGX_EDGE_SHORT", 1) != 0;
    k.edge_pct = env_int("MGX_EDGE_PCT", 23);
    k.last_pct = env_int("MGX_LAST_PCT", 38);
    k.min_chunk = std::max(8, env_int("MGX_MIN_CHUNK", 16));
    k.min_rounds = std::max(1, env_int("MGX_MIN_ROUNDS", 1));
    k.min_rounds_rows = env_int("MGX_MIN_ROUNDS_ROWS", 1024);
    k.pair = env_int("MGX_PAIR", 1) != 0;
    k.pair_ratio = std::max(100, env_int("MGX_PAIR_RATIO", 130));
    k.pair_max_rows = env_int("MGX_PAIR_MAX_ROWS", 640);
    k.pair_min_rows = env_int("MGX_PAIR_MIN_ROWS", 150);
    return k;
}
template <typename T, int K, int PRE, int POST, int SM, int AR>
int launch_cycle_k(const T* vin, const T* b, T* vout, const FoldArgs& fa, int N, long pitch, T c0, T c1, int R,
                   hipStream_t st)
{
    constexpr int OUT = cycle_out_lanes<K, POST, VecOf<T>::W>();
    constexpr bool BL = cycle_b_in_lds<T, K, POST, SM>();
    constexpr int E = (POST == 1 ? 3 : (POST == 2 ? 2 : 0)) + (cycle_skew<T, K, PRE, POST, SM, AR>() > 0 ? 1 : 0);
    constexpr int kTripSteps = BL ? kBRing : trip_steps<T>();
    const int row_lo = fa.row_lo, row_hi = fa.row_hi;
    const CycleWin& win = fa.win;
    if (POST == 1 && !(row_lo & 1)) return -1;
    const int strips = (N / VecOf<T>::W + OUT - 1) / OUT;
    const bool auto_rows = R < 0;
    if (auto_rows) R = -R;
    constexpr int ETOP = POST ? 1 : 0, EBOT = POST == 1 ? 2 : (POST == 2 ? 1 : 0);
    const bool top_edge = (row_lo - K - ETOP) < std::max(win.row_first, 1) || (PRE && ((row_lo - K - ETOP) >> 1) < win.crow_first);
    const bool bot_edge = (row_hi + K + EBOT - 1) > std::min(win.row_last, N - 1) || (PRE && ((row_hi + K + EBOT) >> 1) > win.crow_last);
    GeomKnobs kn = BL ? geom_knobs() : GeomKnobs();
    if (sizeof(T) == 4 && BL) kn.pair_min_rows = std::min(kn.pair_min_rows, env_int("MGX_PAIR_MIN_ROWS_F32", 100));
    const CycleGeom g = cycle_geom_pick(row_lo, row_hi, strips, 2 * K + E, kTripSteps, R, auto_rows, BL, kn, top_edge, bot_edge);
    const int blocks = g.blocks;
    const T w = (fa.restrict_mode == MGX_RESTRICT_FW16) ? (T)0.0625 : (T)0.25;
    hipLaunchKernelGGL((k_jacobi_cycle<T, K, PRE, POST, SM, AR>), dim3(blocks), dim3(kBlock), 0, st, vin, b, vout,
                       (const T*)fa.coarse_e, (T*)fa.coarse_b, (T*)fa.coarse_zero, w, fa.partial, N, pitch, fa.cpitch,
                       row_lo, row_hi, g.R, strips, g.chunks, g.Re, g.chunks_e, g.row_last0, g.Rl, g.RB, g.n_tall, g.n_short, g.Rf, c0, c1, fa.zero_in, win);
    return blocks;
}

template <typename T, int PRE, int POST, int SM, int AR>
int launch_cycle(int K, const T* vin, const T* b, T* vout, const FoldArgs& fa, int N, long pitch, T c0, T c1, int R,
                 hipStream_t st)
{
    switch (K) {
        case 2: return launch_cycle_k<T, 2, PRE, POST, SM, AR>(vin, b, vout, fa, N, pitch, c0, c1, R, st);
        case 4: return launch_cycle_k<T, 4, PRE, POST, SM, AR>(vin, b, vout, fa, N, pitch, c0, c1, R, st);
        case 6: return launch_cycle_k<T, 6, PRE, POST, SM, AR>(vin, b, vout, fa, N, pitch, c0, c1, R, st);
        default: break;
    }
    if constexpr (sizeof(T) == 8 || PRE == 1 || POST == 0) {
        if (K == 8) return launch_cycle_k<T, 8, PRE, POST, SM, AR>(vin, b, vout, fa, N, pitch, c0, c1, R, st);
    }
    if constexpr (!(PRE == 1 && POST == 1) && !(SM == 1 && POST == 1) && !(sizeof(T) == 4 && PRE == 1 && POST == 2) &&
                  !(sizeof(T) == 4 && POST == 1 && AR == 0)) {
        if (K == 10) return launch_cycle_k<T, 10, PRE, POST, SM, AR>(vin, b, vout, fa, N, pitch, c0, c1, R, st);
    }
    if constexpr (SM == 0) {
        switch (K) {
            case 1: return launch_cycle_k<T, 1, PRE, POST, 0, AR>(vin, b, vout, fa, N, pitch, c0, c1, R, st);
            case 3: return launch_cycle_k<T, 3, PRE, POST, 0, AR>(vin, b, vout, fa, N, pitch, c0, c1, R, st);
            case 5: return launch_cycle_k<T, 5, PRE, POST, 0, AR>(vin, b, vout, fa, N, pitch, c0, c1, R, st);
            default: break;
        }
    }
    return -1;
}

template <int PRE_, int POST_> struct Stages { static constexpr int PRE = PRE_, POST = POST_; };
template <typename F>
int with_stages(bool pre, int post, F&& f)
{
    if (pre) return post == 2 ? f(Stages<1, 2>{}) : (post == 1 ? f(Stages<1, 1>{}) : f(Stages<1, 0>{}));
    return post == 2 ? f(Stages<0, 2>{}) : (post == 1 ? f(Stages<0, 1>{}) : f(Stages<0, 0>{}));
}

template <typename T, int SM, int PRE, int POST, int AR>
int launch_tile(const T* vin, const T* b, T* vout, const FoldArgs& fa, int N, long pitch, T c0, T c1, int levels,
                hipStream_t st)
{
    const int He = levels + tile_extra<POST>();
    const int TH = kTileSY - 2 * He, TW = kTileSX - 2 * He;
    if (TH < 8 || TW < 8) return -1;
    const int row_lo = fa.row_lo, row_hi = fa.row_hi;
    const CycleWin& win = fa.win;
    const int tiles_y = (row_hi - row_lo + TH - 1) / TH, tiles_x = (N - 1 + TW - 1) / TW;
    if (tiles_y < 1) return 0;
    const T w = (fa.restrict_mode == MGX_RESTRICT_FW16) ? (T)0.0625 : (T)0.25;
    hipLaunchKernelGGL((k_tile_smooth<T, SM, PRE, POST, AR>), dim3(tiles_y * tiles_x), dim3(kBlock), 0, st, vin, b, vout,
                       (const T*)fa.coarse_e, (T*)fa.coarse_b, (T*)fa.coarse_zero, w, fa.partial, N, pitch, fa.cpitch,
                       levels, c0, c1, tiles_x, fa.zero_in, row_lo, row_hi, win);
    return tiles_y * tiles_x;
}

template <typename T, int SM, int PRE, int POST, int AR>
int launch_tile_wide(const T* vin, const T* b, T* vout, const FoldArgs& fa, int N, long pitch, T c0, T c1, int levels,
                     int rw, hipStream_t st)
{
    if (VecOf<T>::W == 4) rw = 8;
    const int row_lo = fa.row_lo, row_hi = fa.row_hi;
    const CycleWin& win = fa.win;
    const TileWideGeom g = tile_wide_geom(N, row_lo, row_hi, levels + tile_extra<POST>(), VecOf<T>::W, rw);
    if (g.TH < 8 || g.TW < 8) return -1;
    if (g.tiles_y < 1) return 0;
    const T w = (fa.restrict_mode == MGX_RESTRICT_FW16) ? (T)0.0625 : (T)0.25;
    const dim3 grid(g.tiles_y * g.tiles_x), block(kTileWideWaves * kWave);
    if (rw == 8)
        hipLaunchKernelGGL((k_tile_wide<T, SM, PRE, POST, AR, 8>), grid, block, 0, st, vin, b, vout, (const T*)fa.coarse_e,
                           (T*)fa.coarse_b, (T*)fa.coarse_zero, w, fa.partial, N, pitch, fa.cpitch, levels, c0, c1, g.tiles_x,
                           fa.zero_in, row_lo, row_hi, win);
    else if constexpr (VecOf<T>::W == 2) {
        if (rw != 10) return -1;
        hipLaunchKernelGGL((k_tile_wide<T, SM, PRE, POST, AR, 10>), grid, block, 0, st, vin, b, vout, (const T*)fa.coarse_e,
                           (T*)fa.coarse_b, (T*)fa.coarse_zero, w, fa.partial, N, pitch, fa.cpitch, levels, c0, c1, g.tiles_x,
                           fa.zero_in, row_lo, row_hi, win);
    } else {
        return -1;
    }
    return g.tiles_y * g.tiles_x;
}

template <typename T, int SM, int AR>
int launch_tile_pass(const T* vin, const T* b, T* vout, const FoldArgs& fa, int N, long pitch, T c0, T c1, int levels,
                     int band, bool pre, int post, hipStream_t st)
{
    return with_stages(pre, post, [&](auto s) {
        using S = decltype(s);
        return band ? launch_tile_wide<T, SM, S::PRE, S::POST, AR>(vin, b, vout, fa, N, pitch, c0, c1, levels, band, st)
                    : launch_tile<T, SM, S::PRE, S::POST, AR>(vin, b, vout, fa, N, pitch, c0, c1, levels, st);
    });
}

template <typename T>
void launch_restrict(const T* v, const T* b, T* cb, T* czero, int N, long pitch, long cpitch,
                     int crow_lo, int crow_hi, int fine_row_off, int mode, bool fused, int rpc, hipStream_t st)
{
    if (crow_hi <= crow_lo) return;
    Launch g = make_launch(N, VecOf<T>::W, crow_hi - crow_lo, rpc > 0 ? (rpc + 1) / 2 : 0);
    const T w = (mode == MGX_RESTRICT_FW16) ? (T)0.0625 : (T)0.25;
    if (fused)
        hipLaunchKernelGGL((k_restrict<T, true>), dim3(g.blocks), dim3(kBlock), 0, st, v, b, cb, czero, N, pitch,
                           cpitch, crow_lo, crow_hi, fine_row_off, g.R, g.strips, g.chunks, w);
    else
        hipLaunchKernelGGL((k_restrict<T, false>), dim3(g.blocks), dim3(kBlock), 0, st, v, b, cb, czero, N, pitch,
                           cpitch, crow_lo, crow_hi, fine_row_off, g.R, g.strips, g.chunks, w);
}

template <typename T>
void launch_prolong(T* v, const T* e, int N, long pitch, long cpitch, int row_lo, int row_hi,
                    int fine_row_off, bool add, int rpc, hipStream_t st)
{
    if (row_hi <= row_lo) return;
    const Launch g = make_launch(N, VecOf<T>::W, row_hi - row_lo, rpc);
    if (add)
        hipLaunchKernelGGL((k_prolong<T, true>), dim3(g.blocks), dim3(kBlock), 0, st, v, e, N, pitch, cpitch,
                           row_lo, row_hi, fine_row_off, g.R, g.strips, g.chunks);
    else
        hipLaunchKernelGGL((k_prolong<T, false>), dim3(g.blocks), dim3(kBlock), 0, st, v, e, N, pitch, cpitch,
                           row_lo, row_hi, fine_row_off, g.R, g.strips, g.chunks);
}

template <typename T> long sumsq_blocks(int N, int rows, int rpc)
{
    return make_launch(N, VecOf<T>::W, rows, rpc).blocks;
}

template <typename T, int MODE>
void launch_residual(const T* v, const T* b, void* out, long pitch_out, double* partial, double* sum_dev,
                     double inv_scale, int N, long pitch, int row_lo, int row_hi, int rpc, hipStream_t st,
                     long partial_cap, int rows_alloc)
{
    Launch g = make_launch(N, VecOf<T>::W, row_hi - row_lo, rpc);
    if (MODE != 0 && partial_cap >= 0 && g.blocks > partial_cap) {
        const int R = (int)(((long)g.strips * (row_hi - row_lo) / kWavesPerBlock + partial_cap - 9) / (partial_cap - 8)) + 1;
        g = make_launch(N, VecOf<T>::W, row_hi - row_lo, R);
    }
    hipLaunchKernelGGL((k_residual<T, MODE>), dim3(g.blocks), dim3(kBlock), 0, st, v, b, out, pitch_out, partial,
                       inv_scale, N, pitch, row_lo, row_hi, g.R, g.strips, g.chunks, rows_alloc);
    if (MODE != 0)
        hipLaunchKernelGGL(k_reduce_partials, dim3(1), dim3(kReduceThreads), 0, st, partial, g.blocks, sum_dev);
}


#define MGX_FOR_SMAR(X, T) X(T, 0, 0) X(T, 0, 1) X(T, 1, 0)
#define MGX_DECL_CYCLE_PP(T, PRE, POST, SM, AR) \
    extern template int launch_cycle<T, PRE, POST, SM, AR>(int, const T*, const T*, T*, const FoldArgs&, int, long, T, T, int, hipStream_t);
#define MGX_DECL_CYCLE(T, SM, AR) MGX_DECL_CYCLE_PP(T, 1, 2, SM, AR) MGX_DECL_CYCLE_PP(T, 1, 0, SM, AR) MGX_DECL_CYCLE_PP(T, 0, 1, SM, AR) \
    MGX_DECL_CYCLE_PP(T, 0, 2, SM, AR) MGX_DECL_CYCLE_PP(T, 1, 1, SM, AR)
#define MGX_DECL_FUSED(T, SM, AR) \
    extern template bool launch_fused<T, SM, AR>(int, const T*, const T*, T*, int, long, int, int, T, T, int, int, int, int, hipStream_t, int, int);
#define MGX_DECL_TILE(T, SM, AR) \
    extern template int launch_tile_pass<T, SM, AR>(const T*, const T*, T*, const FoldArgs&, int, long, T, T, int, int, bool, int, hipStream_t);
#if !defined(MGX_INST_KIND) && !defined(MGX_SINGLE_TU)
MGX_FOR_SMAR(MGX_DECL_CYCLE, double) MGX_FOR_SMAR(MGX_DECL_CYCLE, float)
MGX_FOR_SMAR(MGX_DECL_FUSED, double) MGX_FOR_SMAR(MGX_DECL_FUSED, float)
MGX_FOR_SMAR(MGX_DECL_TILE, double) MGX_FOR_SMAR(MGX_DECL_TILE, float)
#endif

}
```

### multigrid_nikhil_c-_amd/csrc/mgx_pass_plan.hpp

```cpp
#pragma once

#include "../../include/mgx.h"
#include "mgx_geom.hpp"

#include <algorithm>
#include <cstdlib>
#include <vector>

namespace mgx {

inline int env_int(const char* name, int dflt)
{
    const char* s = getenv(name);
    return (s && *s) ? atoi(s) : dflt;
}

struct FuseCfg {
    int kmax; int rows; int min_n; int fold_kmax; int fold_kmax_big; int tile_max_n; int tile_k; int fold_kmax_nopost;
    int tile_wide; int tile_short_n;
    int plan_pre[8] = {0}; int n_pre = 0; int plan_post[8] = {0}; int n_post = 0; int plan_min_n = 8192;
    int arith = 0;
};

inline int fuse_rows_deep(int N, int rows)
// ... 68 lines not shown
    return f;
}

inline bool cycle_k_supported(int K, bool rbgs, bool f64, int post, bool pre, int arith)
{
    if (K == 10) return !(pre && post == 1) && !(rbgs && post == 1) && !(!f64 && pre && post == 2) && !(!f64 && post == 1 && arith == 0);
    if (K == 8 && !f64 && !pre && post != 0) return false;
    return rbgs ? (K == 2 || K == 4 || K == 6 || K == 8) : (K >= 1 && K <= 8 && K != 7);
}

inline bool fused_k_supported(int K, bool rbgs)
{
    return K == 2 || K == 4 || K == 6 || K == 8 || K == 10 || (!rbgs && (K == 3 || K == 5));
}

inline int tile_band(const FuseCfg& fc, int N, bool f64)
{
    return (fc.tile_wide >= (f64 ? 1 : 2)) ? tile_wide_rw(N, fc.tile_short_n) : 0;
}

constexpr double kFuseRate64[11] = {0, 1.00, 1.80, 2.45, 3.16, 3.81, 4.80, 0, 5.60, 0, 5.63};
constexpr double kFuseRate32[11] = {0, 1.00, 1.67, 2.38, 3.10, 3.77, 4.26, 0, 4.98, 0, 4.67};
constexpr double kFuseRateGS64[11] = {0, 1.00, 1.81, 2.50, 3.19, 3.12, 0, 0, 0, 0, 0};
constexpr double kFuseRateGS32[11] = {0, 1.00, 1.79, 2.20, 2.87, 2.69, 0, 0, 0, 0, 0};

inline double fold_pass_cost(int K, bool rbgs, int post, bool f64, int arith)
{
    if (!cycle_k_supported(K, rbgs, f64, post, false, arith)) return -1.0;
    if (rbgs) return K <= 4 ? 1.0 : (K == 6 ? 1.1 : (K == 8 ? 1.3 : 2.4));
    if (K <= 5) return 1.0;
    if (!f64) return K == 6 ? 1.34 : (K == 8 ? 1.53 : 1.75);
    if (K == 6) return 1.05;
    if (K == 8) return 1.12;
    return 1.46;
}

template <typename Cost>
std::vector<int> split_sweeps(int mu, int smax, double launch, double eps, Cost cost)
{
    std::vector<double> best(mu + 1, 1e300);
    std::vector<int> pick(mu + 1, 1);
    best[0] = 0.0;
    for (int m = 1; m <= mu; ++m)
        for (int k = 1; k <= std::min(m, smax); ++k) {
            const double c = cost(k, m);
            if (c < 0.0) continue;
            const double t = best[m - k] + c + launch;
            if (t < best[m] - eps) { best[m] = t; pick[m] = k; }
        }
    std::vector<int> parts;
    for (int m = mu; m > 0; m -= pick[m]) parts.push_back(pick[m]);
    return parts;
}

enum PassKind {
    PASS_JACOBI,
    PASS_RBGS,
    PASS_FUSED,
    PASS_FOLDED,
    PASS_TILE,
};

struct Pass {
    int kind;
    int K;
    bool pre; int post;
    bool zero_in;
    int lo, hi;
    int R;
};

struct BlockReq {
    int smoother = MGX_SMOOTHER_JACOBI; bool f64 = true;
    int N = 0, row0 = 0, rows = 0;
    int row_lo = 0, row_hi = 0;
    int mu = 0;
    bool pre = false;
    int post = 0;
    bool zero_in = false;
    bool widen = true;
    bool strict = false;
    long tile_points = 0;
    int rpc = 0;
};

inline bool fold_plan(const FuseCfg& fc, const BlockReq& q, std::vector<Pass>* plan)
{
    plan->clear();
    const bool rbgs = (q.smoother == MGX_SMOOTHER_RBGS);
    const int per = rbgs ? 2 : 1, N = q.N, mu = q.mu;
    const int first = 1 - q.row0, last = N - q.row0;
    {
        const int lo = std::max(std::max(q.row_lo, first), 1), hi = std::min(std::min(q.row_hi, last), q.rows - 1);
        const bool whole = q.row_lo <= first && q.row_hi >= last;
        if (fc.tile_max_n > 0 && hi > lo && (long)(hi - lo) * N <= q.tile_points && (per * mu <= fc.tile_k || whole)) {
            const int smax = std::max(1, fc.tile_k / per), np = (mu + smax - 1) / smax;
            for (int p = 0; p < np; ++p) {
                const int sw = mu / np + (p < mu % np ? 1 : 0);
                plan->push_back({PASS_TILE, per * sw, q.pre && p == 0, p == np - 1 ? q.post : 0, q.zero_in && p == 0,
                                 lo + q.row0, hi + q.row0, tile_band(fc, N, q.f64)});
            }
            return true;
        }
    }
    const bool staged = q.pre || q.post != 0;
    const bool fuse = fc.kmax > per && N >= fc.min_n && (q.row_hi - q.row_lo) >= 64 && mu <= 64;
    std::vector<int> parts;
    if (!staged) {
        const double* rate = rbgs ? (q.f64 ? kFuseRateGS64 : kFuseRateGS32) : (q.f64 ? kFuseRate64 : kFuseRate32);
        if (fuse)
            parts = split_sweeps(mu, std::max(1, std::min(fc.kmax, 10) / per), 0.02, 0.0,
                                 [&](int k, int) { return rate[k] > 0.0 ? (double)k / rate[k] : -1.0; });
        else
            parts.assign(std::max(mu, 0), 1);
    } else {
        const int* forced = nullptr;
        int nf = 0;
        if (!q.pre && q.post == 1) { forced = fc.plan_pre; nf = fc.n_pre; }
        else if (q.pre) { forced = fc.plan_post; nf = fc.n_post; }
        if (nf > 0 && N >= fc.plan_min_n) {
            int sum = 0;
            bool ok = true;
            for (int i = 0; i < nf; ++i) {
                sum += forced[i];
                const int K = per * forced[i];
                const bool folded = (i == 0 && q.pre) || (i == nf - 1 && q.post != 0);
                const int Q = (i == nf - 1) ? q.post : 0;
                ok = ok && K <= 10 && (folded ? cycle_k_supported(K, rbgs, q.f64, Q, q.pre && i == 0, fc.arith) : (K != 7 && K != 9 && (!rbgs || K % 2 == 0)));
            }
            if (ok && sum == mu) parts.assign(forced, forced + nf);
        }
        if (parts.empty()) {
            int kcap = N >= 8192 ? fc.fold_kmax_big : fc.fold_kmax;
            if (q.post == 0) kcap = std::min(kcap, fc.fold_kmax_nopost);
            if (rbgs) kcap = std::min(kcap, env_int("MGX_FOLD_KMAX_GS", 10));
            if (q.pre && q.post == 1) kcap = std::min(kcap, 8);
            parts = split_sweeps(mu, std::max(1, kcap / per), 1e-3, 1e-12, [&](int k, int m) {
                if (k == mu && m == mu && !cycle_k_supported(per * k, rbgs, q.f64, q.post, q.pre, fc.arith)) return -1.0;
                return fold_pass_cost(per * k, rbgs, q.post, q.f64, fc.arith);
            });
            std::sort(parts.begin(), parts.end(), [](int a, int b) { return a > b; });
        }
    }
    const int np = (int)parts.size();
    const int stage_rows = q.post == 2 ? 1 : (q.post == 1 ? 2 : 0);
    int done = 0;
    for (int p = 0; p < np; ++p) {
        const int sw = parts[p], K = per * sw;
        const bool P = q.pre && p == 0, zin = q.zero_in && p == 0;
        const int Q = (p == np - 1) ? q.post : 0;
        const int ext = q.widen ? per * (mu - (done + sw)) + (p != np - 1 ? stage_rows : 0) : 0;
        int lo = std::max(q.row_lo - ext, first), hi = std::min(q.row_hi + ext, last);
        if (q.strict && hi > lo && (std::max(lo - K, first - 1) < 0 || std::min(hi + K - 1, last) > q.rows - 1)) return false;
        lo = std::max(lo, 1);
        hi = std::min(hi, q.rows - 1);
        const int kind = (P || Q) ? PASS_FOLDED : (!rbgs && K == 1) ? PASS_JACOBI : (rbgs && !staged && !fuse) ? PASS_RBGS : PASS_FUSED;
        int R = q.rpc;
        if (kind == PASS_FUSED || kind == PASS_FOLDED) R = fuse_rows(fc, N, K, q.f64, hi - lo);
        if (hi > lo) {
            if (kind == PASS_FOLDED) {
                if (!cycle_k_supported(K, rbgs, q.f64, Q, P, fc.arith)) return false;
                if (Q == 1 && !((lo + q.row0) & 1)) return false;
                if (fuse_rows_auto(fc, N, K, q.f64)) R = -R;
            }
            if (kind == PASS_FUSED && !fused_k_supported(K, rbgs)) return false;
            if (zin && (kind == PASS_JACOBI || kind == PASS_RBGS)) return false;
        }
// ... 8 lines not shown
```

Before: 1161 billion.

## Fuse initial residual norm into first descend smoothing pass and use mapped host sum

Adds an N0 template variant of the folded Jacobi cycle kernel that computes the initial residual norm partials while doing the first pre-smoothing and restriction, so the separate initial residual-norm sweep over the fine grid is skipped. The initial norm is read asynchronously through an event while the coarse part of the first cycle is enqueued, and the first cycle is rolled back if the tolerance is already met. The reduction kernel also writes the sum straight to a mapped host pointer, which removes the device-to-host memcpy per norm. This costs an extra kernel instantiation and a more complex first-cycle control path.

```diff
diff --git a/multigrid_nikhil_c-_amd/csrc/mgx.hip b/multigrid_nikhil_c-_amd/csrc/mgx.hip
--- a/multigrid_nikhil_c-_amd/csrc/mgx.hip
+++ b/multigrid_nikhil_c-_amd/csrc/mgx.hip
@@ -69,6 +69,7 @@
     long partial_cap = 0;
     double* sum_dev = nullptr;
     double* sum_host = nullptr;
+    double* sum_mirror = nullptr;
     std::string err;
     int rows_per_chunk = 0;
     FuseCfg fuse{10, 0, 256, 10, 10, 1024, 10, 10};
@@ -80,6 +81,8 @@
     int fold = 1;
     int use_zero_in = 1;
     int norm_blocks_ready = 0;
+    int norm0 = 1;
+    hipEvent_t norm0_ev = nullptr;
     double fine_updates = 0.0;
     struct CycleGraph {
         std::vector<void*> before, after;
@@ -546,7 +549,7 @@
         hipLaunchKernelGGL((k_residual_var<T, decltype(nq)::value, MODE>), dim3(g.blocks), dim3(kBlock), 0, s->stream, (const T*)u, (const T*)b,
                            (T*)out, s->partial, v.a, v.N, v.pitch, 1, v.N, g.strips, v.rows);
     });
-    if (MODE == 1) hipLaunchKernelGGL(k_reduce_partials, dim3(1), dim3(kReduceThreads), 0, s->stream, s->partial, g.blocks, s->sum_dev);
+    if (MODE == 1) hipLaunchKernelGGL(k_reduce_partials, dim3(1), dim3(kReduceThreads), 0, s->stream, s->partial, g.blocks, s->sum_dev, s->sum_mirror);
 }
 
 template <int MODE>
@@ -556,7 +559,8 @@
         using T = decltype(tag);
         if (s->var) residual_var_t<T, MODE>(s, l, u, b, out);
         else launch_residual<T, MODE>((const T*)u, (const T*)b, out, MODE ? 0 : l.pitch, MODE ? s->partial : nullptr, MODE ? s->sum_dev : nullptr,
-                                      1.0, l.N, l.pitch, 1, l.N, s->rows_per_chunk, s->stream, MODE ? s->partial_cap : -1, l.rows);
+                                      1.0, l.N, l.pitch, 1, l.N, s->rows_per_chunk, s->stream, MODE ? s->partial_cap : -1, l.rows,
+                                      MODE ? s->sum_mirror : nullptr);
     });
 }
 
@@ -567,6 +571,9 @@
 {
     std::vector<Pass> plan;
     if (!fold_plan(fc, q, &plan)) return -1;
+    if (q.norm0 && !(SM == 0 && plan.size() == 1 && plan[0].kind == PASS_FOLDED && !plan[0].pre && plan[0].post == 1 &&
+                     plan[0].hi > plan[0].lo && norm0_k_supported(plan[0].K, q.f64, AR)))
+        return -1;
     const int N = q.N, row0 = q.row0;
     const JacobiCoef<T> jc = jacobi_coef<T>(omega);
     FoldArgs fa;
@@ -602,7 +609,10 @@
             else if (p.kind == PASS_FUSED)
                 rc = launch_fused<T, SM, AR>(p.K, src, b, dst, N, pitch, lo, hi, jc.c0, jc.c1, -row0, N - row0, row0 & 1, p.R, st,
                                              q.rows, fa.zero_in) ? 0 : -1;
-            else if (p.kind == PASS_FOLDED)
+            else if (p.kind == PASS_FOLDED && q.norm0) {
+                if constexpr (SM == 0) rc = launch_cycle<T, 0, 1, 0, AR, 1>(p.K, src - back, b - back, dst - back, fa, N, pitch, jc.c0, jc.c1, p.R, st);
+                else rc = -1;
+            } else if (p.kind == PASS_FOLDED)
                 rc = with_stages(p.pre, p.post, [&](auto s) {
                     using S = decltype(s);
                     if constexpr (S::PRE || S::POST)
@@ -613,7 +623,7 @@
             else
                 rc = launch_tile_pass<T, SM, AR>(src - back, b - back, dst - back, fa, N, pitch, jc.c0, jc.c1, p.K, p.R, p.pre, p.post, st);
             if (rc < 0) return -1;
-            if (p.post == 2) blocks = rc;
+            if (p.post == 2 || q.norm0) blocks = rc;
         }
         std::swap(src, dst);
     }
@@ -637,7 +647,7 @@
     return fold_eligible(s, s->lv[level], s->cfg.mu1, false, 1, true);
 }
 
-bool smooth_folded(mgx_solver* s, int level, int mu, bool pre, int post, bool zero_in = false, bool coarse_zero_in = false)
+bool smooth_folded(mgx_solver* s, int level, int mu, bool pre, int post, bool zero_in = false, bool coarse_zero_in = false, bool norm0 = false)
 {
     Level& l = s->lv[level];
     if (!fold_eligible(s, l, mu, pre, post)) return false;
@@ -652,7 +662,8 @@
         const int dt = l.f64 ? MGX_DTYPE_F64 : MGX_DTYPE_F32;
         const mgx_slab cs{level - 1, dt, c.rows, 0, s->cfg.arith};
         void* czero = (post == 1 && coarse_zero_in) ? nullptr : c.u;
-        const BlockReq q = level_req(s, l, mu, pre, post, zero_in, env_int("MGX_ROWS", 0));
+        BlockReq q = level_req(s, l, mu, pre, post, zero_in, env_int("MGX_ROWS", 0));
+        q.norm0 = norm0;
         int launches = 0;
         const int nb = with_kernel_set(l.f64, s->cfg.smoother, s->fuse.arith, [&](auto k) {
             using K = decltype(k);
@@ -664,7 +675,7 @@
         if (nb < 0) return false;
         if (launches & 1) std::swap(l.u, l.tmp);
         p.set(launches, mu);
-        if (post == 2) s->norm_blocks_ready = nb;
+        if (post == 2 || norm0) s->norm_blocks_ready = nb;
     }
     if (fine) s->fine_updates += (double)mu * (double)(l.N - 1) * (double)(l.N - 1);
     return true;
@@ -772,10 +783,10 @@
     return MGX_OK;
 }
 
-bool descend(mgx_solver* s, int level, bool zero_in_here)
+bool descend(mgx_solver* s, int level, bool zero_in_here, bool norm0 = false)
 {
     const bool zin_next = zero_in_ok(s, level - 1);
-    if (!smooth_folded(s, level, s->cfg.mu1, false, 1, zero_in_here, zin_next)) {
+    if (!smooth_folded(s, level, s->cfg.mu1, false, 1, zero_in_here, zin_next, norm0)) {
         if (zero_in_here) (void)zero_u(s, level);
         smooth(s, level, s->cfg.mu1);
         restrict_level(s, level, true, !zin_next);
@@ -889,13 +900,13 @@
     if (s->norm_blocks_ready > 0 && u == s->lv[s->cfg.finest_level].u && !s->mixed) {
         Prof p(s, cls, 1);
         hipLaunchKernelGGL(k_reduce_partials, dim3(1), dim3(kReduceThreads), 0, s->stream, s->partial, s->norm_blocks_ready,
-                           s->sum_dev);
+                           s->sum_dev, s->sum_mirror);
     } else {
         Prof p(s, cls, 2);
         residual_level<1>(s, l, u, b, nullptr);
     }
     s->norm_blocks_ready = 0;
-    HIPCHK(s, hipMemcpyAsync(s->sum_host, s->sum_dev, sizeof(double), hipMemcpyDeviceToHost, s->stream));
+    if (!s->sum_mirror) HIPCHK(s, hipMemcpyAsync(s->sum_host, s->sum_dev, sizeof(double), hipMemcpyDeviceToHost, s->stream));
     return MGX_OK;
 }
 
@@ -1020,6 +1031,56 @@
     return MGX_OK;
 }
 
+bool norm0_ok(const mgx_solver* s, double tol, int max_cycles)
+{
+    const int L = s->cfg.finest_level;
+    if (!s->norm0 || s->dist || s->mixed || s->var || s->cfg.schedule == MGX_SCHEDULE_FMG) return false;
+    if (s->cfg.smoother != MGX_SMOOTHER_JACOBI || L <= s->cfg.coarsest_level) return false;
+    if (max_cycles < 1 || !(tol < 1.0)) return false;
+    const Level& l = s->lv[L];
+    if (!fold_eligible(s, l, s->cfg.mu1, false, 1)) return false;
+    std::vector<Pass> plan;
+    if (!fold_plan(s->fuse, level_req(s, l, s->cfg.mu1, false, 1, false, env_int("MGX_ROWS", 0)), &plan)) return false;
+    return plan.size() == 1 && plan[0].kind == PASS_FOLDED && !plan[0].pre && plan[0].post == 1 && plan[0].hi > plan[0].lo &&
+           norm0_k_supported(plan[0].K, l.f64, s->fuse.arith);
+}
+
+int norm0_first_cycle(mgx_solver* s, double tol, double* r0, double* r1, bool* ran)
+{
+    const int L = s->cfg.finest_level;
+    const bool split = s->use_graph && s->cfg.profile != 1;
+    if (!s->norm0_ev) HIPCHK(s, hipEventCreateWithFlags(&s->norm0_ev, hipEventDisableTiming));
+    const std::vector<void*> before = buffer_state(s);
+    s->norm_blocks_ready = 0;
+    const bool zin_next = descend(s, L, false, true);
+    if (s->norm_blocks_ready <= 0) return s->fail(MGX_ERR_STATE, "the descend pass with the input-norm stage did not run as planned");
+    if (int rc = enqueue_norm(s, s->lv[L], s->lv[L].u, s->lv[L].b, MGX_PROF_NORM_FINE)) return rc;
+    HIPCHK(s, hipEventRecord(s->norm0_ev, s->stream));
+    struct Chain {
+        mgx_solver* s;
+        Chain(mgx_solver* s_, bool on) : s(s_) { s->prof_chain = on && env_int("MGX_PROF_CHAIN", 1) != 0; s->chain_ev = nullptr; }
+        ~Chain() { s->prof_chain = false; s->chain_ev = nullptr; }
+    } chain(s, s->cfg.profile == 2 && split);
+    if (split) {
+        if (int rc = coarse_part_graph(s, L - 1, zin_next)) return rc;
+    } else {
+        coarse_visits(s, L - 1, zin_next, s->cycle);
+    }
+    HIPCHK(s, hipEventSynchronize(s->norm0_ev));
+    *r0 = std::sqrt(*s->sum_host);
+    *ran = !(*r0 <= tol * *r0);
+    if (!*ran) {
+        set_buffer_state(s, before);
+        s->fine_updates = 0.0;
+        return MGX_OK;
+    }
+    ascend(s, L, 2);
+    if (int rc = enqueue_norm(s, s->lv[L], s->lv[L].u, s->lv[L].b, MGX_PROF_NORM_FINE)) return rc;
+    HIPCHK(s, hipStreamSynchronize(s->stream));
+    *r1 = std::sqrt(*s->sum_host);
+    return MGX_OK;
+}
+
 void finish_solve(mgx_stats* stats, double* history, int history_cap, const std::vector<double>& hist, int cycles, bool converged,
                   std::chrono::steady_clock::time_point t0, double fine_updates)
 {
@@ -1219,6 +1280,7 @@
     s->fuse.arith = cfg->arith;
     s->fold = env_int("MGX_FOLD", 1);
     s->use_zero_in = env_int("MGX_ZERO_IN", 1);
+    s->norm0 = env_int("MGX_NORM0", 1);
     s->use_graph = env_int("MGX_GRAPH", 1);
     s->small_visit = env_int("MGX_SMALL_VISIT", 1);
     s->line_dirs = cfg->smoother == MGX_SMOOTHER_LINE_X ? 1 : cfg->smoother == MGX_SMOOTHER_LINE_Y ? 2 : cfg->smoother == MGX_SMOOTHER_LINE_ALT ? 3 : 0;
@@ -1288,6 +1350,11 @@
             s->err = "allocation of reduction buffers failed";
             return bail(MGX_ERR_ALLOC);
         }
+        *s->sum_host = 0.0;
+        if (env_int("MGX_HOST_SUM", 1) && hipHostGetDevicePointer((void**)&s->sum_mirror, s->sum_host, 0) != hipSuccess) {
+            (void)hipGetLastError();
+            s->sum_mirror = nullptr;
+        }
     }
     if (cfg->bottom == MGX_BOTTOM_EXACT && !var) {
         if (s->bottom.init((1 << cfg->coarsest_level) - 1) != hipSuccess) {
@@ -1316,6 +1383,7 @@
     s->kry.free();
     drop_graphs(s);
     for (auto& p : s->ev_used) { (void)hipEventDestroy(p.a); (void)hipEventDestroy(p.b); }
+    if (s->norm0_ev) (void)hipEventDestroy(s->norm0_ev);
     for (auto& p : s->ev_free) { (void)hipEventDestroy(p.a); (void)hipEventDestroy(p.b); }
     if (s->stream) (void)hipStreamDestroy(s->stream);
     delete s;
@@ -1799,9 +1867,20 @@
 
     if (!s->mixed) {
         Level& l = s->lv[L];
-        if ((rc = residual_norm_grid(s, l, l.u, l.b, &r, MGX_PROF_NORM_FINE))) return rc;
-        hist.push_back(r);
-        for (k = 0; k < max_cycles; ++k) {
+        if (norm0_ok(s, tol, max_cycles)) {
+            double r1 = 0.0;
+            bool ran = false;
+            if ((rc = norm0_first_cycle(s, tol, &r, &r1, &ran))) return rc;
+            hist.push_back(r);
+            if (ran) {
+                hist.push_back(r1);
+                k = 1;
+            }
+        } else {
+            if ((rc = residual_norm_grid(s, l, l.u, l.b, &r, MGX_PROF_NORM_FINE))) return rc;
+            hist.push_back(r);
+        }
+        for (; k < max_cycles; ++k) {
             if (hist[k] <= tol * hist[0]) break;
             s->norm_blocks_ready = 0;
             if (k == 0 && do_fmg) {
@@ -1862,14 +1941,14 @@
                     hipLaunchKernelGGL(k_update_residual, dim3(gr.blocks), dim3(kBlock), 0, s->stream, (const double*)d.u,
                                        (const float*)w.u, (const double*)d.b, (double*)d.tmp, (float*)w.b, pending_scale,
                                        1.0 / next_scale, s->partial, d.N, d.pitch, w.pitch, 1, d.N, gr.R, gr.strips, gr.chunks);
-                    hipLaunchKernelGGL(k_reduce_partials, dim3(1), dim3(kReduceThreads), 0, s->stream, s->partial, gr.blocks, s->sum_dev);
+                    hipLaunchKernelGGL(k_reduce_partials, dim3(1), dim3(kReduceThreads), 0, s->stream, s->partial, gr.blocks, s->sum_dev, s->sum_mirror);
                     std::swap(d.u, d.tmp);
                 } else {
                     launch_residual<double, 2>((const double*)d.u, (const double*)d.b, w.b, w.pitch, s->partial,
-                                               s->sum_dev, 1.0 / next_scale, d.N, d.pitch, 1, d.N, rpc, s->stream, s->partial_cap, d.rows);
+                                               s->sum_dev, 1.0 / next_scale, d.N, d.pitch, 1, d.N, rpc, s->stream, s->partial_cap, d.rows, s->sum_mirror);
                 }
             }
-            HIPCHK(s, hipMemcpyAsync(s->sum_host, s->sum_dev, sizeof(double), hipMemcpyDeviceToHost, s->stream));
+            if (!s->sum_mirror) HIPCHK(s, hipMemcpyAsync(s->sum_host, s->sum_dev, sizeof(double), hipMemcpyDeviceToHost, s->stream));
             HIPCHK(s, hipStreamSynchronize(s->stream));
             hist.push_back(std::sqrt(*s->sum_host));
         }
@@ -2050,7 +2129,7 @@
                                            (T*)coarse_b, nullptr, crow_lo, crow_hi, restrict_mode, scratch, st, &flips);
     });
     if (nb < 0) return MGX_ERR_INVALID;
-    if (post == 2) hipLaunchKernelGGL(k_reduce_partials, dim3(1), dim3(kReduceThreads), 0, st, scratch, nb, sum_dev);
+    if (post == 2) hipLaunchKernelGGL(k_reduce_partials, dim3(1), dim3(kReduceThreads), 0, st, scratch, nb, sum_dev, (double*)nullptr);
     if (result_in_tmp) *result_in_tmp = flips & 1;
     return hipGetLastError() == hipSuccess ? MGX_OK : MGX_ERR_HIP;
 }
diff --git a/multigrid_nikhil_c-_amd/csrc/mgx_inst.hip b/multigrid_nikhil_c-_amd/csrc/mgx_inst.hip
--- a/multigrid_nikhil_c-_amd/csrc/mgx_inst.hip
+++ b/multigrid_nikhil_c-_amd/csrc/mgx_inst.hip
@@ -20,10 +20,16 @@
 #define PP_ 0, 1
 #elif MGX_INST_PP == 3
 #define PP_ 0, 2
+#elif MGX_INST_PP == 5
+#define PP_ 0, 1
+#define N0_ 1
 #else
 #define PP_ 1, 1
 #endif
-template int launch_cycle<T_, PP_, MGX_INST_SM, MGX_INST_AR>(int, const T_*, const T_*, T_*, const FoldArgs&, int, long, T_, T_, int, hipStream_t);
+#ifndef N0_
+#define N0_ 0
+#endif
+template int launch_cycle<T_, PP_, MGX_INST_SM, MGX_INST_AR, N0_>(int, const T_*, const T_*, T_*, const FoldArgs&, int, long, T_, T_, int, hipStream_t);
 #elif MGX_INST_KIND == 2
 template bool launch_fused<T_, MGX_INST_SM, MGX_INST_AR>(int, const T_*, const T_*, T_*, int, long, int, int, T_, T_, int, int, int, int, hipStream_t, int, int);
 #elif MGX_INST_KIND == 3
diff --git a/multigrid_nikhil_c-_amd/csrc/mgx_kernels.hpp b/multigrid_nikhil_c-_amd/csrc/mgx_kernels.hpp
--- a/multigrid_nikhil_c-_amd/csrc/mgx_kernels.hpp
+++ b/multigrid_nikhil_c-_amd/csrc/mgx_kernels.hpp
@@ -658,7 +658,7 @@
 }
 
 constexpr int kReduceThreads = 1024;
-static __global__ void __launch_bounds__(kReduceThreads) k_reduce_partials(const double* __restrict__ partial, int n, double* __restrict__ out)
+static __global__ void __launch_bounds__(kReduceThreads) k_reduce_partials(const double* __restrict__ partial, int n, double* __restrict__ out, double* __restrict__ out_host)
 {
     __shared__ double wsum[kReduceThreads / kWave];
     double a0 = 0.0, a1 = 0.0, a2 = 0.0, a3 = 0.0;
@@ -678,6 +678,7 @@
         double s = 0.0;
         for (int w = 0; w < kReduceThreads / kWave; ++w) s += wsum[w];
         out[0] = s;
+        if (out_host) out_host[0] = s;
     }
 }
 
@@ -947,7 +948,7 @@
 #ifndef MGX_RAWQ
 #define MGX_RAWQ 1
 #endif
-template <typename T, int K, int PRE, int POST, int SM, int AR> constexpr bool cycle_rawq();
+template <typename T, int K, int PRE, int POST, int SM, int AR, int N0 = 0> constexpr bool cycle_rawq();
 template <typename T> struct LdsVec;
 template <> struct LdsVec<double> { typedef double v __attribute__((ext_vector_type(2))); };
 template <> struct LdsVec<float> { typedef float v __attribute__((ext_vector_type(4))); };
@@ -973,11 +974,12 @@
     return make_float4(t.x, t.y, t.z, t.w);
 }
 constexpr int ring_slot(int m) { return ((m % kBRing) + kBRing) % kBRing; }
-template <typename T, int K, int PRE, int POST, int SM, int AR> constexpr bool cycle_rawq()
+template <typename T, int K, int PRE, int POST, int SM, int AR, int N0> constexpr bool cycle_rawq()
 {
     if (MGX_RAWQ == 0) return false;
     if (PRE != 0 || sizeof(T) != 8) return false;
     if (POST == 2 && AR == 0 && K == 10) return false;
+    if (N0 != 0 && AR == 0 && K == 10) return false;
     return cycle_b_in_lds<T, K, POST, SM>() && SM == 0 && POST != 0 && K > kRawLds && cycle_skew<T, K, PRE, POST, SM, AR>() == 0;
 }
 #ifndef MGX_PFD_DEEP
@@ -991,10 +993,10 @@
 constexpr int kPrefetchMax = MGX_PFD_DEEP > kPrefetch ? MGX_PFD_DEEP : kPrefetch;
 template <typename T, bool BL, bool EDGE, int POST> constexpr int cycle_cpfd() { return (BL && !(EDGE && POST == 0)) ? cycle_pfd<BL, POST, EDGE>() : 1; }
 
-template <typename T, int K, int PRE, int POST, int SM, bool EDGE, int RP, bool BL, bool ZIN, int AR, int YP>
+template <typename T, int K, int PRE, int POST, int SM, bool EDGE, int RP, bool BL, bool ZIN, int AR, int YP, int N0 = 0>
 __device__ __forceinline__ void
 cycle_step(typename VecOf<T>::type (&lev)[K + 1][3], typename VecOf<T>::type (&bw)[BL ? 1 : K + 1], lds_vec_ptr<T> ring,
-           lds_vec_ptr<T> ring2, typename VecOf<T>::type (&rawq)[cycle_rawq<T, K, PRE, POST, SM, AR>() ? kBRing : 1],
+           lds_vec_ptr<T> ring2, typename VecOf<T>::type (&rawq)[cycle_rawq<T, K, PRE, POST, SM, AR, N0>() ? kBRing : 1],
            typename VecOf<T>::type (&nin)[kPfStages], typename VecOf<T>::type (&nbn)[kPfStages], PreFetch<T, VecOf<T>::W / 2>& pe,
            CycleState<T, VecOf<T>::W / 2>& cs, int y,
            const T* __restrict__ pv, const T* __restrict__ pb, T* __restrict__ po,
@@ -1071,7 +1073,7 @@
         if constexpr (W == 2) { in.x = in.x + add.x; in.y = in.y + add.y; }
         else { in.x = in.x + add.x; in.y = in.y + add.y; in.z = in.z + add.z; in.w = in.w + add.w; }
     }
-    constexpr bool RAWQ = cycle_rawq<T, K, PRE, POST, SM, AR>();
+    constexpr bool RAWQ = cycle_rawq<T, K, PRE, POST, SM, AR, N0>();
     constexpr bool PREMUL = (SM == 0 && POST == 0) || RAWQ;
     V b0;
     if constexpr (PREMUL) b0 = vscale(c1, bn);
@@ -1102,6 +1104,21 @@
     };
     V dying = lev[SK][S_NEW];
     lev[0][S_NEW] = in;
+    if constexpr (N0) {
+        static_assert(PRE == 0 && POST == 1 && SM == 0, "the input-norm stage rides on the plain descend pass");
+        V res0 = residual_vec(lev[0][S_OLD], lev[0][S_MID], lev[0][S_NEW], bn);
+        int row = y - 1;
+        if constexpr (EDGE) {
+            row = opaque_s(y - 1);
+            mask_sel(res0, cm, !(row > bnd_lo && row < bnd_hi));
+        }
+        double q2;
+        if constexpr (W == 2) q2 = (double)res0.x * (double)res0.x + (double)res0.y * (double)res0.y;
+        else q2 = ((double)res0.x * (double)res0.x + (double)res0.y * (double)res0.y) +
+                  ((double)res0.z * (double)res0.z + (double)res0.w * (double)res0.w);
+        cs.acc += (st && row >= r0 && row < r1) ? q2 : 0.0;
+        if constexpr (EDGE) asm volatile("" : "+v"(cs.acc));
+    }
     auto level = [&](auto jc, auto bc) {
         constexpr int j = decltype(jc)::value;
         constexpr bool inB = decltype(bc)::value;
@@ -1225,7 +1242,7 @@
     }
 }
 
-template <typename T, int K, int PRE, int POST, int SM, bool EDGE, bool ZIN, int AR>
+template <typename T, int K, int PRE, int POST, int SM, bool EDGE, bool ZIN, int AR, int N0 = 0>
 __device__ __forceinline__ double
 cycle_body(const T* __restrict__ pv, const T* __restrict__ pb, T* __restrict__ po,
            const T* __restrict__ coarse_e, T* __restrict__ coarse_b, T* __restrict__ coarse_zero, T wgt,
@@ -1233,7 +1250,7 @@
            const CycleWin& win, lds_vec_ptr<T> ring, lds_vec_ptr<T> ring2, const FastOut& fo)
 {
     constexpr bool BL = cycle_b_in_lds<T, K, POST, SM>();
-    constexpr bool RAWQ = cycle_rawq<T, K, PRE, POST, SM, AR>();
+    constexpr bool RAWQ = cycle_rawq<T, K, PRE, POST, SM, AR, N0>();
     using V = typename VecOf<T>::type;
     constexpr int W = VecOf<T>::W;
     constexpr int CW = W / 2;
@@ -1294,7 +1311,7 @@
                 if (((PAR + q) & 1) == 1) coarse_row<T, EDGE>(pe[q].b, ((y0 + q) >> 1) + 1, cld, ca.win, fo);
         }
     }
-#define MGX_CSTEP(RP, Y) cycle_step<T, K, PRE, POST, SM, EDGE, RP, BL, ZIN, AR, (PAR < 0 ? -1 : ((PAR + (RP)) & 1))>(lev, bw, ring, ring2, rawq, nin[(RP) % PFD], nbn[(RP) % PFD], pe[(RP) % CPFD], cs, Y, pv, pb, po, coarse_e, coarse_b, coarse_zero, wgt, pitch, col, ccol, N, ca, ld, cld, st, c0, c1, fo)
+#define MGX_CSTEP(RP, Y) cycle_step<T, K, PRE, POST, SM, EDGE, RP, BL, ZIN, AR, (PAR < 0 ? -1 : ((PAR + (RP)) & 1)), N0>(lev, bw, ring, ring2, rawq, nin[(RP) % PFD], nbn[(RP) % PFD], pe[(RP) % CPFD], cs, Y, pv, pb, po, coarse_e, coarse_b, coarse_zero, wgt, pitch, col, ccol, N, ca, ld, cld, st, c0, c1, fo)
     if constexpr (BL) {
 #define MGX_CTRIP(Y) do { MGX_CSTEP(0, Y); MGX_CSTEP(1, Y + 1); MGX_CSTEP(2, Y + 2); MGX_CSTEP(3, Y + 3); MGX_CSTEP(4, Y + 4); \
                           MGX_CSTEP(5, Y + 5); MGX_CSTEP(6, Y + 6); MGX_CSTEP(7, Y + 7); MGX_CSTEP(8, Y + 8); MGX_CSTEP(9, Y + 9); \
@@ -1333,7 +1350,7 @@
 {
     return cycle_b_in_lds<T, K, POST, SM>() ? 2 : 1;
 }
-template <typename T, int K, int PRE, int POST, int SM = 0, int AR = 0>
+template <typename T, int K, int PRE, int POST, int SM = 0, int AR = 0, int N0 = 0>
 __global__ void __launch_bounds__(kBlock, (cycle_waves<T, K, PRE, POST, SM, AR>()))
 k_jacobi_cycle(const T* __restrict__ vin, const T* __restrict__ rhs, T* __restrict__ vout,
                const T* __restrict__ coarse_e,
@@ -1351,7 +1368,7 @@
     __shared__ double wsum[kWavesPerBlock];
     constexpr bool BL = cycle_b_in_lds<T, K, POST, SM>();
     __shared__ typename LdsVec<T>::v bring[BL ? kWavesPerBlock * kBRing * kWave : 1];
-    constexpr bool RAWQ = cycle_rawq<T, K, PRE, POST, SM, AR>();
+    constexpr bool RAWQ = cycle_rawq<T, K, PRE, POST, SM, AR, N0>();
     __shared__ typename LdsVec<T>::v braw[RAWQ ? kWavesPerBlock * kRawLds * kWave : 1];
     const CTile t = cycle_tile(strips, chunks, chunks_e, R, Re, row_lo, row_hi, row_last0, Rl, RB, n_tall, n_short, Rf);
     double acc = 0.0;
@@ -1397,13 +1414,13 @@
         fo.clane_off = (unsigned)((col / 2) * (long)sizeof(T));
         if (interior) {
             if (PRE == 0 && zero_in)
-                acc = cycle_body<T, K, PRE, POST, SM, false, PRE == 0, AR>(vin + col, rhs + col, vout + col, coarse_e, coarse_b, coarse_zero, wgt,
+                acc = cycle_body<T, K, PRE, POST, SM, false, PRE == 0, AR, N0>(vin + col, rhs + col, vout + col, coarse_e, coarse_b, coarse_zero, wgt,
                                                                       pitch, cpitch, col, N, r0, r1, true, st, c0, c1, true, win, ring, ring2, fo);
             else
-                acc = cycle_body<T, K, PRE, POST, SM, false, false, AR>(vin + col, rhs + col, vout + col, coarse_e, coarse_b, coarse_zero, wgt,
+                acc = cycle_body<T, K, PRE, POST, SM, false, false, AR, N0>(vin + col, rhs + col, vout + col, coarse_e, coarse_b, coarse_zero, wgt,
                                                                     pitch, cpitch, col, N, r0, r1, true, st, c0, c1, false, win, ring, ring2, fo);
         } else {
-            acc = cycle_body<T, K, PRE, POST, SM, true, false, AR>(vin + col, rhs + col, vout + col, coarse_e, coarse_b, coarse_zero, wgt,
+            acc = cycle_body<T, K, PRE, POST, SM, true, false, AR, N0>(vin + col, rhs + col, vout + col, coarse_e, coarse_b, coarse_zero, wgt,
                                                         pitch, cpitch, col, N, r0, r1, ld, st, c0, c1, zero_in != 0, win, ring, ring2, fo);
         }
     }
@@ -1420,7 +1437,7 @@
         if (w == 0) g_wave_trace_n = gridDim.x * kWavesPerBlock;
     }
 #endif
-    if (POST == 2) {
+    if (POST == 2 || N0) {
         for (int off = 32; off > 0; off >>= 1) acc += __shfl_down(acc, off, kWave);
         if ((threadIdx.x & 63) == 0) wsum[threadIdx.x >> 6] = acc;
         __syncthreads();
diff --git a/multigrid_nikhil_c-_amd/csrc/mgx_launch.hpp b/multigrid_nikhil_c-_amd/csrc/mgx_launch.hpp
--- a/multigrid_nikhil_c-_amd/csrc/mgx_launch.hpp
+++ b/multigrid_nikhil_c-_amd/csrc/mgx_launch.hpp
@@ -128,7 +128,7 @@
     k.pair_min_rows = env_int("MGX_PAIR_MIN_ROWS", 150);
     return k;
 }
-template <typename T, int K, int PRE, int POST, int SM, int AR>
+template <typename T, int K, int PRE, int POST, int SM, int AR, int N0 = 0>
 int launch_cycle_k(const T* vin, const T* b, T* vout, const FoldArgs& fa, int N, long pitch, T c0, T c1, int R,
                    hipStream_t st)
 {
@@ -150,34 +150,34 @@
     const CycleGeom g = cycle_geom_pick(row_lo, row_hi, strips, 2 * K + E, kTripSteps, R, auto_rows, BL, kn, top_edge, bot_edge);
     const int blocks = g.blocks;
     const T w = (fa.restrict_mode == MGX_RESTRICT_FW16) ? (T)0.0625 : (T)0.25;
-    hipLaunchKernelGGL((k_jacobi_cycle<T, K, PRE, POST, SM, AR>), dim3(blocks), dim3(kBlock), 0, st, vin, b, vout,
+    hipLaunchKernelGGL((k_jacobi_cycle<T, K, PRE, POST, SM, AR, N0>), dim3(blocks), dim3(kBlock), 0, st, vin, b, vout,
                        (const T*)fa.coarse_e, (T*)fa.coarse_b, (T*)fa.coarse_zero, w, fa.partial, N, pitch, fa.cpitch,
                        row_lo, row_hi, g.R, strips, g.chunks, g.Re, g.chunks_e, g.row_last0, g.Rl, g.RB, g.n_tall, g.n_short, g.Rf, c0, c1, fa.zero_in, win);
     return blocks;
 }
 
-template <typename T, int PRE, int POST, int SM, int AR>
+template <typename T, int PRE, int POST, int SM, int AR, int N0 = 0>
 int launch_cycle(int K, const T* vin, const T* b, T* vout, const FoldArgs& fa, int N, long pitch, T c0, T c1, int R,
                  hipStream_t st)
 {
     switch (K) {
-        case 2: return launch_cycle_k<T, 2, PRE, POST, SM, AR>(vin, b, vout, fa, N, pitch, c0, c1, R, st);
-        case 4: return launch_cycle_k<T, 4, PRE, POST, SM, AR>(vin, b, vout, fa, N, pitch, c0, c1, R, st);
-        case 6: return launch_cycle_k<T, 6, PRE, POST, SM, AR>(vin, b, vout, fa, N, pitch, c0, c1, R, st);
+        case 2: return launch_cycle_k<T, 2, PRE, POST, SM, AR, N0>(vin, b, vout, fa, N, pitch, c0, c1, R, st);
+        case 4: return launch_cycle_k<T, 4, PRE, POST, SM, AR, N0>(vin, b, vout, fa, N, pitch, c0, c1, R, st);
+        case 6: return launch_cycle_k<T, 6, PRE, POST, SM, AR, N0>(vin, b, vout, fa, N, pitch, c0, c1, R, st);
         default: break;
     }
     if constexpr (sizeof(T) == 8 || PRE == 1 || POST == 0) {
-        if (K == 8) return launch_cycle_k<T, 8, PRE, POST, SM, AR>(vin, b, vout, fa, N, pitch, c0, c1, R, st);
+        if (K == 8) return launch_cycle_k<T, 8, PRE, POST, SM, AR, N0>(vin, b, vout, fa, N, pitch, c0, c1, R, st);
     }
     if constexpr (!(PRE == 1 && POST == 1) && !(SM == 1 && POST == 1) && !(sizeof(T) == 4 && PRE == 1 && POST == 2) &&
                   !(sizeof(T) == 4 && POST == 1 && AR == 0)) {
-        if (K == 10) return launch_cycle_k<T, 10, PRE, POST, SM, AR>(vin, b, vout, fa, N, pitch, c0, c1, R, st);
+        if (K == 10) return launch_cycle_k<T, 10, PRE, POST, SM, AR, N0>(vin, b, vout, fa, N, pitch, c0, c1, R, st);
     }
     if constexpr (SM == 0) {
         switch (K) {
-            case 1: return launch_cycle_k<T, 1, PRE, POST, 0, AR>(vin, b, vout, fa, N, pitch, c0, c1, R, st);
-            case 3: return launch_cycle_k<T, 3, PRE, POST, 0, AR>(vin, b, vout, fa, N, pitch, c0, c1, R, st);
-            case 5: return launch_cycle_k<T, 5, PRE, POST, 0, AR>(vin, b, vout, fa, N, pitch, c0, c1, R, st);
+            case 1: return launch_cycle_k<T, 1, PRE, POST, 0, AR, N0>(vin, b, vout, fa, N, pitch, c0, c1, R, st);
+            case 3: return launch_cycle_k<T, 3, PRE, POST, 0, AR, N0>(vin, b, vout, fa, N, pitch, c0, c1, R, st);
+            case 5: return launch_cycle_k<T, 5, PRE, POST, 0, AR, N0>(vin, b, vout, fa, N, pitch, c0, c1, R, st);
             default: break;
         }
     }
@@ -285,7 +285,7 @@
 template <typename T, int MODE>
 void launch_residual(const T* v, const T* b, void* out, long pitch_out, double* partial, double* sum_dev,
                      double inv_scale, int N, long pitch, int row_lo, int row_hi, int rpc, hipStream_t st,
-                     long partial_cap, int rows_alloc)
+                     long partial_cap, int rows_alloc, double* sum_host = nullptr)
 {
     Launch g = make_launch(N, VecOf<T>::W, row_hi - row_lo, rpc);
     if (MODE != 0 && partial_cap >= 0 && g.blocks > partial_cap) {
@@ -295,7 +295,7 @@
     hipLaunchKernelGGL((k_residual<T, MODE>), dim3(g.blocks), dim3(kBlock), 0, st, v, b, out, pitch_out, partial,
                        inv_scale, N, pitch, row_lo, row_hi, g.R, g.strips, g.chunks, rows_alloc);
     if (MODE != 0)
-        hipLaunchKernelGGL(k_reduce_partials, dim3(1), dim3(kReduceThreads), 0, st, partial, g.blocks, sum_dev);
+        hipLaunchKernelGGL(k_reduce_partials, dim3(1), dim3(kReduceThreads), 0, st, partial, g.blocks, sum_dev, sum_host);
 }
 
 
@@ -304,12 +304,15 @@
     extern template int launch_cycle<T, PRE, POST, SM, AR>(int, const T*, const T*, T*, const FoldArgs&, int, long, T, T, int, hipStream_t);
 #define MGX_DECL_CYCLE(T, SM, AR) MGX_DECL_CYCLE_PP(T, 1, 2, SM, AR) MGX_DECL_CYCLE_PP(T, 1, 0, SM, AR) MGX_DECL_CYCLE_PP(T, 0, 1, SM, AR) \
     MGX_DECL_CYCLE_PP(T, 0, 2, SM, AR) MGX_DECL_CYCLE_PP(T, 1, 1, SM, AR)
+#define MGX_DECL_CYCLE_N0(T, AR) \
+    extern template int launch_cycle<T, 0, 1, 0, AR, 1>(int, const T*, const T*, T*, const FoldArgs&, int, long, T, T, int, hipStream_t);
 #define MGX_DECL_FUSED(T, SM, AR) \
     extern template bool launch_fused<T, SM, AR>(int, const T*, const T*, T*, int, long, int, int, T, T, int, int, int, int, hipStream_t, int, int);
 #define MGX_DECL_TILE(T, SM, AR) \
     extern template int launch_tile_pass<T, SM, AR>(const T*, const T*, T*, const FoldArgs&, int, long, T, T, int, int, bool, int, hipStream_t);
 #if !defined(MGX_INST_KIND) && !defined(MGX_SINGLE_TU)
 MGX_FOR_SMAR(MGX_DECL_CYCLE, double) MGX_FOR_SMAR(MGX_DECL_CYCLE, float)
+MGX_DECL_CYCLE_N0(double, 0) MGX_DECL_CYCLE_N0(double, 1) MGX_DECL_CYCLE_N0(float, 0) MGX_DECL_CYCLE_N0(float, 1)
 MGX_FOR_SMAR(MGX_DECL_FUSED, double) MGX_FOR_SMAR(MGX_DECL_FUSED, float)
 MGX_FOR_SMAR(MGX_DECL_TILE, double) MGX_FOR_SMAR(MGX_DECL_TILE, float)
 #endif
diff --git a/multigrid_nikhil_c-_amd/csrc/mgx_pass_plan.hpp b/multigrid_nikhil_c-_amd/csrc/mgx_pass_plan.hpp
--- a/multigrid_nikhil_c-_amd/csrc/mgx_pass_plan.hpp
+++ b/multigrid_nikhil_c-_amd/csrc/mgx_pass_plan.hpp
@@ -174,7 +174,13 @@
     bool strict = false;
     long tile_points = 0;
     int rpc = 0;
-};
+    bool norm0 = false;
+};
+
+inline bool norm0_k_supported(int K, bool f64, int arith)
+{
+    return cycle_k_supported(K, false, f64, 1, false, arith);
+}
 
 inline bool fold_plan(const FuseCfg& fc, const BlockReq& q, std::vector<Pass>* plan)
 {
```

New measurement: 1157 billion. No clear change (-0.3%).
